# A-Nasiri-M/sap3d_tensorflow

Hardware: AMD Instinct MI355X
Metric: clips/s (16x112x112 fwd+bwd) (higher is better)
Workload: dtype f32

## Files before the change

### include/p3d_hip.h

```cpp
#ifndef P3D_HIP_H
#define P3D_HIP_H
#include <stddef.h>
#include <stdint.h>

#ifdef __cplusplus
extern "C" {
#endif

typedef struct p3d_handle p3d_handle;

enum {
    P3D_STRUCTURE_UNET = 0,
    P3D_STRUCTURE_CONCAT = 1,
    P3D_STRUCTURE_GN_P3D = 2,
    P3D_STRUCTURE_UNETPP_NONSA = 3,
    P3D_STRUCTURE_GN_P3D_DECODER = 4,
    P3D_STRUCTURE_GN_P3D_CONCAT = 5,
    P3D_STRUCTURE_UNETPP_DS = 6
};

typedef struct p3d_config {
    int structure;
    int batch;
    int frames;
// ... 104 lines not shown
typedef struct p3d_op_time {
    char name[64];
    char kernel[48];
    double ms;
    double flops;
    double bytes;
    int phase;
} p3d_op_time;
int p3d_profile_step(p3d_handle* h, float dropout_rate, uint64_t seed, p3d_op_time* out, int cap);

#define P3D_COMM_ID_BYTES 128
int p3d_comm_unique_id(void* id_out);
int p3d_comm_init(p3d_handle* h, const void* id);
int p3d_device_count(void);
int p3d_comm_info(p3d_handle* h, int* n_ranks, int* rank, int* device);
int p3d_debug_bucket_audit(p3d_handle* h, float dropout_rate, uint64_t seed, int64_t bucket_floats, int64_t* lo, int64_t* hi,
                           int32_t* after_op, int cap, int64_t* n_train, int64_t* stale);

int64_t p3d_debug_dirty_counters(void);

int p3d_debug_install_abort_trace(void);

int p3d_debug_force_plan(int igemm_tile, int igemm_splits, int wgrad_tm, int wgrad_tn);

int p3d_op_conv3d(int device, const float* x, const int64_t xshape[5], const float* w, const int64_t wshape[5],
                  const int s[3], const float* bias, float* y);
int p3d_op_conv3d_backprop_input(int device, const float* dy, const float* w, const int64_t wshape[5],
                                 const int s[3], const int64_t xshape[5], float* dx);
int p3d_op_conv3d_backprop_filter(int device, const float* x, const int64_t xshape[5], const float* dy,
                                  const int64_t wshape[5], const int s[3], float* dw, float* dbias);
int p3d_op_conv3d_transpose(int device, const float* x, const int64_t xshape[5], const float* k,
                            const int64_t kshape[5], const int s[3], const float* bias, float* y);
int p3d_debug_stem_wgrad_through_bn(int device, const float* x, const int64_t xshape[5], const float* y, const float* dz, const float* tab,
                                    const float* coef, int batch, float* dw_fused, float* dw_two_launches);
int p3d_debug_conv_bn_stats(int device, const float* x, const int64_t xshape[5], const float* w, const float* w2, const int64_t wshape[5],
                            const int s[3], const float* bias, int transpose, float* moving, float* y, float* y2, float* stats,
                            int* nparts, const char** kernel);
int p3d_debug_bn_pass(int device, int mode, int64_t M, int C, const float* y1, int ld1, int off1, const float* y2, int ld2, int off2,
                      const float* params, int batch1, int batch2, int update_moving, const float* dz, int acc2, float drop_rate,
                      uint64_t seed, int seed_dev, int path, float* z, int ldz, int offz, float* dy1, float* dy2, float* grads,
                      float* moving, int* info);
int p3d_debug_gn_pass(int device, int mode, int N, int R, int C, int G, float eps, const float* y1, int ld1, const float* y2, int ld2,
                      int ldz, const float* params, const float* cs, const float* ss, const float* dz, int acc2, float drop_rate,
                      uint64_t seed, int path, float* z, float* dy1, float* dy2, float* grads, float* tables, int* info);
int p3d_debug_cbam(int device, int N, int D, int H, int W, int C, const float* x, int ld, const float* k0, const float* b0,
                   const float* k1, const float* b1, const float* k7, int chunks, const float* dout, int accx, float* cs, float* sp,
                   float* ss, float* dx, float* pgrads, int* info);
int p3d_debug_head(int device, int transpose, int N, int D, int H, int W, int C, const float* x, const float* k, const float* bias,
                   int sigmoid, const float* dlogits, int fwd_path, int filter_path, float* logits, float* pred, float* dx, float* dk,
                   float* dbias, int* info);
int p3d_debug_smooth_l1(int device, const float* pred, const float* target, int64_t n, int through_sigmoid, int offset, double* loss,
                        float* dlogits, int* info);
int p3d_debug_loss(int device, int kind, const float* logits, const float* pred, const float* target, int64_t n, int through_sigmoid,
                   int offset, double* loss, float* dlogits, int* info);
int p3d_debug_map_loss(int device, const float* logits, const float* pred, const float* target, int64_t maps, int64_t map_elems,
                       int through_sigmoid, int offset, float kld_weight, float cc_weight, double* loss, float* dlogits,
                       double* per_map, int* info);
int p3d_debug_saliency_loss(int device, const float* logits, const float* pred, const float* target, const unsigned char* fix,
                            int64_t maps, int64_t map_elems, int through_sigmoid, int offset, float kld_weight, float cc_weight,
                            float nss_weight, float sim_weight, double* loss, float* dlogits, double* per_map, int* info);
int p3d_debug_adam_decay(int device, float* p, float* g, float* m, float* v, int64_t n, int offset, const int64_t* tile_off,
                         const int64_t* tile_len, const float* tile_c, int ntile, float lr, int64_t t, float b1, float b2, float eps,
                         int lr_on_device, int update, double* term, float* lr_t);
int p3d_debug_adam(int device, float* p, const float* g, float* m, float* v, int64_t n, int offset, float lr, int64_t t, float b1,
                   float b2, float eps, int lr_on_device, float* lr_t);
int p3d_debug_optimizer(int device, int kind, float* p, float* g, float* m, int64_t n, int offset, float lr, float momentum,
                        int use_nesterov, int lr_on_device);
int p3d_debug_optimizer_decay(int device, int kind, float* p, float* g, float* m, int64_t n, int offset, const int64_t* tile_off,
                              const int64_t* tile_len, const float* tile_c, int ntile, float lr, float momentum, int use_nesterov,
                              int lr_on_device, int update, double* term);
int p3d_debug_ema(int device, float* s, const float* p, int64_t n, int offset, float om, int om_on_device);
int p3d_debug_grad_accum(int device, int mode, float* acc, float* g, int64_t n, int offset);
int p3d_debug_augment(int device, const float* x, const float* y, const unsigned char* fix, int B, int T, int H, int W, const int32_t* geom,
                      const float* photo, int offset, float* x_out, float* y_out, unsigned char* fix_out);
int p3d_debug_augment_draw(uint64_t seed, uint64_t g, int H, int W, const p3d_augment* cfg, int32_t geom[6], float photo[2]);
int p3d_debug_opt_scaled(int device, int kind, float* p, float* g, float* m, float* v, int64_t n, int offset, const int64_t* tile_off,
                         const int64_t* tile_len, const float* tile_c, int ntile, float lr, int64_t t, float b1, float b2, float eps,
                         float momentum, int use_nesterov, int lr_on_device, float gscale, double* term, float* lr_t);
int p3d_debug_grad_norm(int device, const float* g, const float* p, int64_t n, int offset, const int64_t* chunk_off,
                        const int64_t* chunk_len, const float* chunk_c, int nchunk, const int64_t* range_lo, const int64_t* range_hi,
                        int nrange, float clip_norm, int max_blocks, double* sumsq, double* norm, float* scale);
int p3d_debug_stat_parts(const int64_t xshape[5], const int64_t wshape[5], const int s[3], int transpose, int* written, int* cap);
int p3d_debug_igemm_groupable(const int64_t xshape[5], const int64_t wshape[5], const int s[3]);
int p3d_op_max_pool3d(int device, const float* x, const int64_t xshape[5], const int ksize[3], const int s[3], float* y);
int p3d_op_max_pool3d_grad(int device, const float* x, const int64_t xshape[5], const int ksize[3], const int s[3],
                           const float* dy, float* dx);
int p3d_op_bias_add_grad(int device, const float* dy, int64_t rows, int channels, float* dbias);
int p3d_debug_conv_launch(int device, int kind, const float* in, int ld_in, int off_in, const int64_t xshape[5], const float* w,
                          const int64_t wshape[5], const int s[3], const float* bias, int accum, int f16, float* out, int ld_out,
                          int off_out, char* kernels, int kernels_cap, int* splits);
int p3d_debug_wgrad_group(int device, int n, const float* const* x, const int* ldx, const int* offx, const int64_t* xs,
                          const float* const* dy, const int* lddy, const int* offdy, const int64_t* ws, const int* s, const int* transpose,
                          float* const* dw, float* const* dbias, int polite, int greedy, char* kernel, int kernel_cap, int* cuts,
                          int* info);
typedef struct p3d_fused_bn {
    const float* y; int ld, off;
    const float* gamma; const float* beta;
    const float* partials; int nparts; int64_t rows; int publish, update_moving;
    float* scale; float* shift; float* mean; float* invstd;
    float* moving_mean; float* moving_var;
} p3d_fused_bn;
typedef struct p3d_fused_bn_grad {
    const float* y; int ld, off;
    const float* gamma; const float* mean; const float* invstd;
    const float* partials; int nparts; int64_t rows; int publish;
    float* coef; float* dgamma; float* dbeta;
} p3d_fused_bn_grad;
typedef struct p3d_fused_gate {
    const float* y; int ld_y, off_y;
    const float* scale; const float* shift; const float* mean; const float* invstd;
    float* out; int ld_out, off_out;
    float* part; int part_rows;
} p3d_fused_gate;
typedef struct p3d_fused_conv {
    int kind;
    int64_t xshape[5]; int64_t wshape[5]; int stride[3];
    const float* w; const float* bias; int f16;
    int at; p3d_fused_bn src[2];
    const float* g; int ld_g, off_g;
    int grad; p3d_fused_bn_grad gbn;
    int ngate; p3d_fused_gate gate[2]; int raw_store, accum;
    float* out; int ld_out, off_out;
    int gpart_rows;
} p3d_fused_conv;
int p3d_debug_fused_conv(int device, p3d_fused_conv* a, char* kernels, int kernels_cap, int* splits);
int p3d_debug_fused_wgrad(int device, int n, const float* const* x, const int* ldx, const int* offx, const int64_t* xs,
                          const float* const* dy, const int* lddy, const int* offdy, const int64_t* ws, const int* s,
                          const int* xt, const float* const* x2, const int* ldx2, const int* offx2, const float* const* xs1,
                          const float* const* xt1, const float* const* xs2, const float* const* xt2, const int* dyt,
                          const float* const* dy2, const int* lddy2, const int* offdy2, const float* const* dcoef,
                          float* const* dw, float* const* dbias, char* kernel, int kernel_cap, int* cuts, int* info);
int p3d_debug_fused_reject(int device, int which, int* error, int* validator);
int p3d_debug_max_pool3d(int device, const float* x, int ldx, int offx, const int64_t xshape[5], const int ksize[3], const int s[3],
                         float* y, int ldy, int offy);
int p3d_debug_max_pool3d_grad(int device, const float* x, int ldx, int offx, const int64_t xshape[5], const int ksize[3], const int s[3],
                              const float* dy, int ldy, int offy, int accumulate, float* dx, const char** kernel);
int p3d_debug_bias_add_grad(int device, const float* dy, int64_t rows, int channels, int ld, int off, float* dbias);
int p3d_op_attention_core(int device, int batch, int n_g, int n_f, int ch, const float* g, const float* f, const float* h,
                          float* o, const float* d_o, float* dg, float* df, float* dh);
int p3d_debug_attention_core(int device, int mode, int batch, int n_g, int n_f, int ch, const float* g, const float* f, const float* h,
                             float* o, const float* d_o, float* dg, float* df, float* dh);
int p3d_debug_attention_splits(int batch, int n_g, int n_f, int ch, int splits[4]);
int p3d_debug_softmax_rows(int device, int backward, int64_t rows, int cols, int ld, float* s, float* d, int guard_rows);
int p3d_debug_attn_mix(int device, int64_t M, int C, const float* r, int ldr, int offr, const float* x, int ldx, int offx, float gamma,
                       float drop_rate, uint64_t seed, int seed_dev, float* z, int ldz, int offz, const float* dz, int accx, float* dr,
                       float* dx, float* dgamma);

int p3d_metric_cc(int device, const float* map1, const float* map2, int n_maps, int n_pix, double* out);
int p3d_metric_sim(int device, const float* map1, const float* map2, int n_maps, int n_pix, double* out);
int p3d_metric_nss(int device, const float* sal, const float* fix, int n_maps, int n_pix, double* out);
int p3d_metric_auc_judd(int device, const float* sal, const float* fix, const float* jitter, int n_maps, int n_pix, double* out);
int p3d_metric_auc_borji(int device, const float* sal, const float* fix, const int* rand_idx, int n_pix, int n_fix, int n_rep,
                         double step_size, double* out);
int p3d_mapf_frames(int device, const unsigned char* bgr, int n, int H0, int W0, const float mean_rgb[3], int H, int W, float* out);
int p3d_mapf_density(int device, const unsigned char* grey, int n, int H0, int W0, int H, int W, float* out);

int p3d_resize_linear(int device, const float* src, int n, int h, int w, int H, int W, float* dst);
int p3d_metric_auc_shuffled(int device, const float* sal, const float* fix, const int* other_idx, int n_pix, int n_fix, int n_rand,
                            int n_rep, double step_size, double* out);
int p3d_eval_last_frames(p3d_handle* h, const unsigned char* density, int Hd, int Wd, const unsigned char* fixation, int H, int W,
                         const double* jitter, const int* borji_idx, const int* n_fix, int n_rep, double step_size, double* out,
                         double* stage_ms);
int p3d_debug_eval_maps(int device, const float* maps, int n_maps, int h, int w, int elem_stride, const unsigned char* density,
                        int Hd, int Wd, const unsigned char* fixation, int H, int W, const double* jitter, const int* borji_idx,
                        const int* n_fix, int n_rep, double step_size, double* out);

// ... 233 lines not shown
```

### sap3d_tensorflow_amd/csrc/conv_igemm2.hip

```cpp
#if !defined(__gfx950__) && !defined(__gfx942__) && defined(__HIP_DEVICE_COMPILE__)
#error "the K-slice exchange (write-through slab stores + relaxed ticket + one-lane acquire) is written for gfx942 / gfx950 cache semantics"
#endif
#include "p3d_kernels.h"
#include "igemm_epilogue.h"
#include <algorithm>
#include <cstddef>
#include <cstdio>
#include <cstring>
#include <cstdlib>
#include <map>
#include <mutex>
#include <tuple>
#include <vector>

typedef float f32x16 __attribute__((ext_vector_type(16)));
typedef unsigned u32x4 __attribute__((ext_vector_type(4)));

namespace {

constexpr int BK = 32;
#ifndef P3D_RING64
#define P3D_RING64 3
#endif
template <int BM, int BN>
struct Ring { static constexpr int stages = (BM >= 128) ? 2 : P3D_RING64; };

template <int AT>
struct ATr {
    static constexpr bool two = (AT == P3D_AT_RELU2 || AT == P3D_AT_GRAD);
    static constexpr int ncoef = AT == P3D_AT_RELU1 ? 2 : AT == P3D_AT_RELU2 ? 4 : AT == P3D_AT_GRAD ? 3 : 0;
};

__device__ __forceinline__ void glds16(const float* gsrc, float* lds_wave_base) {
    __builtin_amdgcn_global_load_lds((const __attribute__((address_space(1))) void*)gsrc,
                                     (__attribute__((address_space(3))) void*)lds_wave_base, 16, 0, 0);
}

template <int N>
__device__ __forceinline__ void wait_vmcnt() {
    asm volatile("s_waitcnt vmcnt(%0)" ::"n"(N) : "memory");
}

template <int LA, bool TWO>
struct ALoad {
    int base[LA];
    int dhw[LA];
    const float* aptr[LA];
    const float* aptr2[TWO ? LA : 1];
    int achunk[LA];
    int t, kc;
    int issued;
};
template <int LB>
struct BLoad {
    int boff[LB];
    int bk[LB];
    bool bok[LB];
    int t, kc, issued;
    const float* w;
};

template <int BM, bool TWO>
__device__ __forceinline__ void a_init(const IgemmArgs& p, const Geo& geo, ALoad<BM / 32, TWO>& st, unsigned m0, unsigned M, int wave, int lane,
                                       int s_begin, int kchunks) {
    constexpr int LA = BM / 32;
    const int a_slot = lane & 7, a_sub = lane >> 3;
#pragma unroll
    for (int i = 0; i < LA; ++i) {
        const int r = (i * 4 + wave) * 8 + a_sub;
        const unsigned m = m0 + r;
        st.base[i] = -1; st.dhw[i] = 0; st.aptr[i] = nullptr;
        if (TWO) st.aptr2[TWO ? i : 0] = nullptr;
        st.achunk[i] = 4 * (a_slot ^ ((r >> 1) & 7));
        if (m < M) {
            const unsigned t1 = p3d_div(m, geo.fGw), gw = m - t1 * (unsigned)geo.Gw;
            const unsigned t2 = p3d_div(t1, geo.fGh), gh = t1 - t2 * (unsigned)geo.Gh;
            const unsigned n = p3d_div(t2, geo.fGd), gd = t2 - n * (unsigned)geo.Gd;
            st.base[i] = (int)n * p.Di * p.Hi * p.Wi;
            st.dhw[i] = (int)(((gd * p.isd) << 20) | ((gh * p.ish) << 10) | (gw * p.isw));
        }
    }
    st.t = s_begin / kchunks; st.kc = s_begin - st.t * kchunks; st.issued = 0;
}
template <int BN, bool WT>
__device__ __forceinline__ void b_init(const IgemmArgs& p, const float* w, BLoad<BN / 32>& st, int n0, int wave, int lane, int s_begin, int kchunks) {
    constexpr int LB = BN / 32;
    st.w = w;
    const int a_slot = lane & 7, a_sub = lane >> 3;
    if (!WT) {
        constexpr int LANES_PER_ROW = BN / 4, ROWS_PER_PIECE = 64 / LANES_PER_ROW;
#pragma unroll
        for (int i = 0; i < LB; ++i) {
            const int kr = (i * 4 + wave) * ROWS_PER_PIECE + lane / LANES_PER_ROW;
            const int nc = n0 + (lane % LANES_PER_ROW) * 4;
            st.bk[i] = kr; st.bok[i] = nc < p.Nc; st.boff[i] = kr * p.Nc + nc;
        }
    } else {
#pragma unroll
        for (int i = 0; i < LB; ++i) {
            const int r = (i * 4 + wave) * 8 + a_sub;
            st.bk[i] = 4 * (a_slot ^ ((r >> 1) & 7));
            st.bok[i] = (n0 + r) < p.Nc;
            st.boff[i] = (n0 + r) * p.K + st.bk[i];
        }
    }
    st.t = s_begin / kchunks; st.kc = s_begin - st.t * kchunks; st.issued = 0;
}

template <int LA, bool TWO>
__device__ __forceinline__ void a_set_tap(const IgemmArgs& p, P3dKTap* taps, ALoad<LA, TWO>& st) {
    const P3dTap tap = p3d_ktap(taps, st.t);
#pragma unroll
    for (int i = 0; i < LA; ++i) {
        const int id = (st.dhw[i] >> 20) + tap.dd, ih = ((st.dhw[i] >> 10) & 1023) + tap.dh, iw = (st.dhw[i] & 1023) + tap.dw;
        const bool ok = st.base[i] >= 0 && (unsigned)id < (unsigned)p.Di && (unsigned)ih < (unsigned)p.Hi &&
                        (unsigned)iw < (unsigned)p.Wi;
        const long long row = (long long)st.base[i] + ((long long)id * p.Hi + ih) * p.Wi + iw;
        st.aptr[i] = ok ? p.x + row * p.ldx + st.achunk[i] : nullptr;
        if (TWO) st.aptr2[TWO ? i : 0] = ok ? p.x2 + row * p.ldx2 + st.achunk[i] : nullptr;
    }
}

template <int BM>
__device__ __forceinline__ void issue_a_dma(const IgemmArgs& p, P3dKTap* taps, float* __restrict__ a_dst, ALoad<BM / 32, false>& st, int nsteps,
                                            int kchunks, bool first, int wave, int lane) {
    constexpr int LA = BM / 32;
    const bool live = st.issued < nsteps;
    if (live && (first || st.kc == 0)) a_set_tap(p, taps, st);
    const int k0 = st.kc * BK;
    const float* zp = p.zeros + 4 * (lane & 7);
#pragma unroll
    for (int i = 0; i < LA; ++i) {
        const bool ok = live && st.aptr[i] != nullptr && (k0 + st.achunk[i]) < p.K;
        glds16(ok ? st.aptr[i] + k0 : zp, a_dst + (i * 4 + wave) * 8 * BK);
    }
    ++st.issued;
    if (++st.kc == kchunks) { st.kc = 0; ++st.t; }
}
template <int BN, bool WT>
__device__ __forceinline__ void issue_b_dma(const IgemmArgs& p, P3dKTap* taps, float* __restrict__ b_dst, BLoad<BN / 32>& st, int nsteps, int kchunks,
                                            int wave, int lane) {
    constexpr int LB = BN / 32;
    const bool live = st.issued < nsteps;
    const int k0 = st.kc * BK;
    const float* zp = p.zeros + 4 * (lane & 7);
    const float* wt = st.w + (long long)taps[live ? st.t : 0].widx * p.K * p.Nc;
    if (!WT) {
#pragma unroll
        for (int i = 0; i < LB; ++i) {
            const bool ok = live && st.bok[i] && (k0 + st.bk[i]) < p.K;
            glds16(ok ? wt + (long long)k0 * p.Nc + st.boff[i] : zp, b_dst + (i * 4 + wave) * 256);
        }
    } else {
#pragma unroll
        for (int i = 0; i < LB; ++i) {
            const bool ok = live && st.bok[i] && (k0 + st.bk[i]) < p.K;
            glds16(ok ? wt + k0 + st.boff[i] : zp, b_dst + (i * 4 + wave) * 8 * BK);
        }
    }
    ++st.issued;
    if (++st.kc == kchunks) { st.kc = 0; ++st.t; }
}

struct AMeta {
    unsigned ok;
    int k0;
};
template <int BM, int AT>
__device__ __forceinline__ void issue_a_raw(const IgemmArgs& p, P3dKTap* taps, float* __restrict__ raw_dst, float* __restrict__ raw2_dst, AMeta& r,
                                            ALoad<BM / 32, ATr<AT>::two>& st, int nsteps, int kchunks, bool first, int wave, int lane) {
    constexpr int LA = BM / 32;
    constexpr bool TWO = ATr<AT>::two;
    const bool live = st.issued < nsteps;
    if (live && (first || st.kc == 0)) a_set_tap(p, taps, st);
    const int k0 = st.kc * BK;
    const float* zp = p.zeros + 4 * (lane & 7);
    r.ok = 0; r.k0 = k0;
#pragma unroll
    for (int i = 0; i < LA; ++i) {
        const bool ok = live && st.aptr[i] != nullptr && (k0 + st.achunk[i]) < p.K;
        r.ok |= (ok ? 1u : 0u) << i;
        glds16(ok ? st.aptr[i] + k0 : zp, raw_dst + (i * 4 + wave) * 8 * BK);
        if (TWO) glds16(ok ? st.aptr2[TWO ? i : 0] + k0 : zp, raw2_dst + (i * 4 + wave) * 8 * BK);
    }
    ++st.issued;
    if (++st.kc == kchunks) { st.kc = 0; ++st.t; }
}
__device__ __forceinline__ float relu_nan(float v) { return v > 0.f ? v : (v != v ? v : 0.f); }
__device__ __forceinline__ float4 relu_affine4(float4 s, float4 u, float4 t) {
    return make_float4(relu_nan(fmaf(s.x, u.x, t.x)), relu_nan(fmaf(s.y, u.y, t.y)), relu_nan(fmaf(s.z, u.z, t.z)),
                       relu_nan(fmaf(s.w, u.w, t.w)));
}
template <int LA, int AT>
struct XIn {
    float4 u[LA];
    float4 v[ATr<AT>::two ? LA : 1];
    float4 c[LA][ATr<AT>::ncoef];
};
template <int BM, int AT>
__device__ __forceinline__ void transform_load(const AMeta& r, const float* __restrict__ raw_src, const float* __restrict__ raw2_src,
                                               const int (&achunk)[BM / 32], const float* __restrict__ tab, int kp,
// ... 170 lines not shown
template <int BM, int BN, bool WT, bool F16, int AT, int K>
struct FusedLoop {
    static __device__ __forceinline__ void run(const IgemmArgs& p, P3dKTap* taps, float* ring, const float* tab, int kp, f32x16 (&acc)[BM / 64][BN / 64],
                                               AMeta (&meta)[Ring<BM, BN>::stages - 1], ALoad<BM / 32, ATr<AT>::two>& sa,
                                               BLoad<BN / 32>& sb, int base, int nsteps, int kchunks, int wave, int lane, int wm, int wn) {
        using L = Lds<BM, BN, AT>;
        constexpr int S = L::STAGES, PERIOD = S * (S - 1);
        if constexpr (K < PERIOD) {
            if (base + K < nsteps) {
                constexpr int RS = (K + 1) % (S - 1);
                pipe_step_fused<BM, BN, WT, F16, AT>(p, taps, ring + ((K + 1) % 2) * L::A_STAGE, ring + L::B_OFF + ((K + S - 1) % S) * L::B_STAGE,
                                                     ring + L::RAW_OFF + RS * L::A_STAGE, ring + L::RAW2_OFF + RS * L::A_STAGE,
                                                     ring + (K % 2) * L::A_STAGE, ring + L::B_OFF + (K % S) * L::B_STAGE, tab, kp, acc,
                                                     meta[RS], sa, sb, nsteps, kchunks, wave, lane, wm, wn);
            }
            FusedLoop<BM, BN, WT, F16, AT, K + 1>::run(p, taps, ring, tab, kp, acc, meta, sa, sb, base, nsteps, kchunks, wave, lane, wm, wn);
        }
    }
};

__device__ __forceinline__ void fold_partials(const float* part_base, int nparts, int C, int k, double& s1, double& s2) {
    const float2* part = reinterpret_cast<const float2*>(part_base) + k;
    float2 v[P3D_FOLD_MAX];
#pragma unroll
    for (int q = 0; q < P3D_FOLD_MAX; ++q) v[q] = part[(size_t)min(q, nparts - 1) * C];
#pragma unroll
    for (int q = 0; q < P3D_FOLD_MAX; ++q)
        if (q < nparts) { s1 += (double)v[q].x; s2 += (double)v[q].y; }
}
__device__ __forceinline__ void bn_fold_channel(const BnFold& f, int k, bool owner, float& sc, float& sh) {
    if (!f.part) { sc = f.scale[k]; sh = f.shift[k]; return; }
    double s1 = 0.0, s2 = 0.0;
    fold_partials(f.part, f.nparts, f.C, k, s1, s2);
    const double mean = s1 * f.inv_m;
    double var = s2 * f.inv_m - mean * mean;
    if (var < 0.0) var = 0.0;
    const float meanf = (float)mean, varf = (float)var;
    const float inv = 1.0f / sqrtf(varf + f.eps);
    sc = f.gamma[k] * inv;
    sh = f.beta[k] - meanf * sc;
    if (owner && f.publish) {
        f.scale[k] = sc; f.shift[k] = sh; f.mean[k] = meanf; f.invstd[k] = inv;
        if (f.update_moving) {
            f.moving_mean[k] -= (f.moving_mean[k] - meanf) * (1.0f - 0.99f);
            f.moving_var[k] -= (f.moving_var[k] - varf) * (1.0f - 0.99f);
        }
    }
}
__device__ __forceinline__ void bn_grad_fold_channel(const BnGradFold& f, int k, bool owner, float& k1, float& k2, float& k3) {
    if (!f.part) { k1 = f.coef[k]; k2 = f.coef[f.C + k]; k3 = f.coef[2 * f.C + k]; return; }
    double sg = 0.0, sgx = 0.0;
    fold_partials(f.part, f.nparts, f.C, k, sg, sgx);
    const float inv = f.invstd[k];
    const float c1 = (float)(sg * f.inv_m), c2 = (float)(sgx * f.inv_m);
    k1 = f.gamma[k] * inv;
    k2 = -k1 * inv * c2;
    k3 = -k1 * c1 - k2 * f.mean[k];
    if (owner && f.publish) {
        f.coef[k] = k1; f.coef[f.C + k] = k2; f.coef[2 * f.C + k] = k3;
        f.dgamma[k] = (float)sgx; f.dbeta[k] = (float)sg;
    }
}

template <int AT>
__device__ __forceinline__ void build_table(const IgemmArgs& p, float* tab, int kp, bool owner) {
    for (int k = threadIdx.x; k < kp; k += 256) {
        if constexpr (AT == P3D_AT_RELU1 || AT == P3D_AT_RELU2) {
            float s = 0.f, t = 0.f;
            if (k < p.K) bn_fold_channel(p.f1, k, owner, s, t);
            tab[k] = s; tab[kp + k] = t;
            if constexpr (AT == P3D_AT_RELU2) {
                float s2 = 0.f, t2 = 0.f;
                if (k < p.K) bn_fold_channel(p.f2, k, owner, s2, t2);
                tab[2 * kp + k] = s2; tab[3 * kp + k] = t2;
            }
        } else if constexpr (AT == P3D_AT_GRAD) {
            float k1 = 0.f, k2 = 0.f, k3 = 0.f;
            if (k < p.K) bn_grad_fold_channel(p.gf, k, owner, k1, k2, k3);
            tab[k] = k1; tab[kp + k] = k2; tab[2 * kp + k] = k3;
        }
    }
}

template <int BM, int BN, bool WT, bool F16, int AT>
__device__ __forceinline__ void igemm2_body(const IgemmArgs& p, const Geo& geo, const int tile_id, const int slice) {
    constexpr int TM = BM / 64, TN = BN / 64;
    constexpr int LA = BM / 32;
    using L = Lds<BM, BN, AT>;
    constexpr int STAGES = L::STAGES;

    P3D_CHAIN_PRIO();
    extern __shared__ __attribute__((aligned(16))) char smem[];
    int* rowIdx = reinterpret_cast<int*>(smem);
    float* ring = reinterpret_cast<float*>(rowIdx + BM);
    float* tab = ring + L::FIXED;

    const int tid = threadIdx.x;
    const int lane = tid & 63;
    const int wave = __builtin_amdgcn_readfirstlane(tid >> 6);
    const int wm = wave >> 1, wn = wave & 1;
    const int h = lane >> 5, l31 = lane & 31;

    const long long M = (long long)p.N * geo.Gd * geo.Gh * geo.Gw;
    const int NT = (p.Nc + BN - 1) / BN;
    const int nsplit = geo.nsplit;
    P3dKTap* taps = geo.taps;
    const int nt = tile_id % NT;
    const int mt = tile_id / NT;
    const long long m0 = (long long)mt * BM;
    const int n0 = nt * BN;
    const int kchunks = (p.K + BK - 1) / BK;
    const int kp = kchunks * BK;
    const float4 bias4 = igemm_bias_prefetch<BN>(geo.bias, n0, p.Nc);

    const unsigned Mu = (unsigned)M, m0u = (unsigned)m0;
    auto fill_row_table = [&]() {
        for (int r = tid; r < BM; r += 256) {
            const unsigned m = m0u + r;
            int ro = -1;
            if (m < Mu) {
                const unsigned t1 = p3d_div(m, geo.fGw), gw = m - t1 * (unsigned)geo.Gw;
                const unsigned t2 = p3d_div(t1, geo.fGh), gh = t1 - t2 * (unsigned)geo.Gh;
                const unsigned n = p3d_div(t2, geo.fGd), gd = t2 - n * (unsigned)geo.Gd;
                const int od = gd * p.osd + geo.ood, oh = gh * p.osh + geo.ooh, ow = gw * p.osw + geo.oow;
                ro = (((int)n * p.Do + od) * p.Ho + oh) * p.Wo + ow;
            }
            rowIdx[r] = ro;
        }
    };
    const int total_steps = geo.ntaps * kchunks;
    const int per = (total_steps + nsplit - 1) / nsplit;
    const int s_begin = slice * per;
    const int s_end = min(total_steps, s_begin + per);
    const int nsteps = max(s_end - s_begin, 0);

    f32x16 acc[TM][TN];
#pragma unroll
    for (int i = 0; i < TM; ++i)
#pragma unroll
        for (int j = 0; j < TN; ++j)
#pragma unroll
            for (int e = 0; e < 16; ++e) acc[i][j][e] = 0.f;

    ALoad<LA, ATr<AT>::two> sa;
    BLoad<BN / 32> sb;
    a_init<BM, ATr<AT>::two>(p, geo, sa, m0u, Mu, wave, lane, s_begin, kchunks);
    b_init<BN, WT>(p, geo.w, sb, n0, wave, lane, s_begin, kchunks);
    if constexpr (AT == P3D_AT_NONE) {
#pragma unroll
        for (int k = 0; k < STAGES - 1; ++k) {
            issue_a_dma<BM>(p, taps, ring + k * L::A_STAGE, sa, nsteps, kchunks, k == 0, wave, lane);
            issue_b_dma<BN, WT>(p, taps, ring + L::B_OFF + k * L::B_STAGE, sb, nsteps, kchunks, wave, lane);
        }
        fill_row_table();
        for (int base = 0; base < nsteps; base += STAGES)
            StepLoop<BM, BN, WT, F16, 0>::run(p, taps, ring, acc, sa, sb, base, nsteps, kchunks, wave, lane, wm, wn);
    } else {
        AMeta meta[STAGES - 1];
        float* raw = ring + L::RAW_OFF;
        float* raw2 = ring + L::RAW2_OFF;
        fill_row_table();
        issue_a_raw<BM, AT>(p, taps, raw, raw2, meta[0], sa, nsteps, kchunks, true, wave, lane);
        if constexpr (STAGES == 3) {
            issue_a_raw<BM, AT>(p, taps, raw + L::A_STAGE, raw2 + L::A_STAGE, meta[1], sa, nsteps, kchunks, false, wave, lane);
            issue_b_dma<BN, WT>(p, taps, ring + L::B_OFF, sb, nsteps, kchunks, wave, lane);
        }
        build_table<AT>(p, tab, kp, tile_id == 0 && slice == 0);
        wait_vmcnt<0>();
        __syncthreads();
        {
            XIn<LA, AT> xin;
            transform_load<BM, AT>(meta[0], raw, raw2, sa.achunk, tab, kp, xin, wave, lane);
            transform_store<BM, AT>(meta[0], xin, ring, wave, lane);
        }
        issue_a_raw<BM, AT>(p, taps, raw, raw2, meta[0], sa, nsteps, kchunks, false, wave, lane);
        issue_b_dma<BN, WT>(p, taps, ring + L::B_OFF + (STAGES - 2) * L::B_STAGE, sb, nsteps, kchunks, wave, lane);
        for (int base = 0; base < nsteps; base += STAGES * (STAGES - 1))
            FusedLoop<BM, BN, WT, F16, AT, 0>::run(p, taps, ring, tab, kp, acc, meta, sa, sb, base, nsteps, kchunks, wave, lane, wm, wn);
    }

    constexpr int LDT = BN + 4;
    constexpr int F4R = BN / 4;
    float* tile = ring;
    float* sred = tile + BM * LDT;
    int* flag = reinterpret_cast<int*>(sred + 2 * 4 * BN * 2);
    wait_vmcnt<0>();
    __syncthreads();
#pragma unroll
    for (int i = 0; i < TM; ++i)
#pragma unroll
        for (int j = 0; j < TN; ++j)
#pragma unroll
            for (int e = 0; e < 16; ++e) {
                const int r = wm * (BM / 2) + i * 32 + (e & 3) + 8 * (e >> 2) + 4 * h;
                tile[r * LDT + wn * (BN / 2) + j * 32 + l31] = acc[i][j][e];
            }
    __syncthreads();

    if (nsplit > 1) {
        float* myslab = geo.slab + ((size_t)tile_id * nsplit + slice) * (BM * BN);
        const auto rs = __builtin_amdgcn_make_buffer_rsrc(myslab, 0, BM * BN * 4, 0x00020000);
#pragma unroll 4
        for (int i = tid; i < BM * F4R; i += 256) {
            const int r = i / F4R, c4 = (i - r * F4R) * 4;
            const float4 v = *reinterpret_cast<const float4*>(tile + r * LDT + c4);
            const u32x4 u = {__float_as_uint(v.x), __float_as_uint(v.y), __float_as_uint(v.z), __float_as_uint(v.w)};
            __builtin_amdgcn_raw_buffer_store_b128(u, rs, (r * BN + c4) * 4, 0, 16);
        }
        wait_vmcnt<0>();
        __syncthreads();
        if (tid == 0) {
            const unsigned ticket = __hip_atomic_fetch_add(geo.cnt + tile_id, 1u, __ATOMIC_RELAXED, __HIP_MEMORY_SCOPE_AGENT);
            const int last = ticket == (unsigned)(nsplit - 1);
            if (last) {
                __builtin_amdgcn_fence(__ATOMIC_ACQUIRE, "agent");
                asm volatile("s_waitcnt vmcnt(0)" ::: "memory");
                geo.cnt[tile_id] = 0;
            }
            *flag = last;
        }
        __syncthreads();
        if (!*flag) return;
        const float* slabs = geo.slab + (size_t)tile_id * nsplit * (BM * BN);
        constexpr int PER_LANE = BM * F4R / 256;
        static_assert(PER_LANE % 4 == 0, "reducer unrolls four tile positions");
#pragma unroll 1
        for (int i0 = 0; i0 < PER_LANE; i0 += 4) {
            float4 v[4];
            const float* src[4];
#pragma unroll
            for (int q = 0; q < 4; ++q) {
                const int i = tid + (i0 + q) * 256;
                const int r = i / F4R, c4 = (i - r * F4R) * 4;
                src[q] = slabs + r * BN + c4;
                v[q] = *reinterpret_cast<const float4*>(src[q]);
            }
            int sidx = 1;
            for (; sidx + 3 < nsplit; sidx += 4) {
                float4 a[4][4];
#pragma unroll
                for (int t = 0; t < 4; ++t)
#pragma unroll
                    for (int q = 0; q < 4; ++q) a[t][q] = *reinterpret_cast<const float4*>(src[q] + (size_t)(sidx + t) * (BM * BN));
#pragma unroll
                for (int t = 0; t < 4; ++t)
#pragma unroll
                    for (int q = 0; q < 4; ++q) { v[q].x += a[t][q].x; v[q].y += a[t][q].y; v[q].z += a[t][q].z; v[q].w += a[t][q].w; }
            }
            for (; sidx < nsplit; ++sidx) {
                float4 a[4];
#pragma unroll
                for (int q = 0; q < 4; ++q) a[q] = *reinterpret_cast<const float4*>(src[q] + (size_t)sidx * (BM * BN));
#pragma unroll
                for (int q = 0; q < 4; ++q) { v[q].x += a[q].x; v[q].y += a[q].y; v[q].z += a[q].z; v[q].w += a[q].w; }
            }
#pragma unroll
            for (int q = 0; q < 4; ++q) {
                const int i = tid + (i0 + q) * 256;
                const int r = i / F4R, c4 = (i - r * F4R) * 4;
                *reinterpret_cast<float4*>(tile + r * LDT + c4) = v[q];
            }
        }
        __syncthreads();
    }

    igemm_tile_epilogue<BM, BN>(p, geo, tile, sred, rowIdx, mt, n0, M, bias4);
}

__device__ __forceinline__ int xcd_tile(int b, int T, int min_tiles) {
    if (T < min_tiles) return b;
    const int x = b & 7, q = T >> 3, r = T & 7;
    return x * q + min(x, r) + (b >> 3);
}

template <int BM, int BN, bool WT, bool F16 = false, int AT = 0>
__global__ __launch_bounds__(256) void igemm2_kernel(const IgemmArgs p) {
    p3d_warm_kernargs<IgemmArgs>();
    Geo geo;
    geo.Gd = p.Gd; geo.Gh = p.Gh; geo.Gw = p.Gw; geo.fGd = p.fGd; geo.fGh = p.fGh; geo.fGw = p.fGw;
    geo.ood = p.ood; geo.ooh = p.ooh; geo.oow = p.oow; geo.stat_base = p.stat_base; geo.ntaps = p.ntaps; geo.taps = p3d_kernarg_taps(offsetof(IgemmArgs, taps));
    geo.w = p.w; geo.bias = p.bias; geo.y = p.y; geo.statpart = p.statpart;
    geo.nsplit = p.nsplit; geo.slab = p.slab; geo.cnt = p.cnt;
    const int tile = p.nsplit == 1 ? xcd_tile((int)blockIdx.x, (int)gridDim.x, p.xcd_min_tiles) : (int)blockIdx.x;
    igemm2_body<BM, BN, WT, F16, AT>(p, geo, tile, (int)blockIdx.y);
}
template <int BM, int BN, bool WT, bool F16 = false>
__global__ __launch_bounds__(256) void igemm2_group_kernel(const IgemmGroupArgs g) {
    p3d_warm_kernargs<IgemmArgs>();
    int c = 0;
#pragma unroll
    for (int q = 1; q < P3D_IGEMM_CLASSES; ++q)
        if (q < g.nclass && (int)blockIdx.x >= g.cls[q].blk0) c = q;
    Geo geo;
    geo.Gd = g.cls[c].Gd; geo.Gh = g.cls[c].Gh; geo.Gw = g.cls[c].Gw; geo.fGd = g.cls[c].fGd; geo.fGh = g.cls[c].fGh; geo.fGw = g.cls[c].fGw;
    geo.ood = g.cls[c].ood; geo.ooh = g.cls[c].ooh; geo.oow = g.cls[c].oow; geo.stat_base = g.cls[c].stat_base; geo.ntaps = g.cls[c].ntaps;
    geo.taps = p3d_kernarg_taps(offsetof(IgemmGroupArgs, cls) + (size_t)c * sizeof(IgemmClass) + offsetof(IgemmClass, taps));
    geo.w = g.cls[c].w; geo.bias = g.cls[c].bias; geo.y = g.cls[c].y; geo.statpart = g.cls[c].statpart;
    const int tile0 = g.cls[c].tile0;
    geo.nsplit = g.cls[c].nsplit;
    geo.slab = g.common.slab + (g.cls[c].slab0 - (long long)tile0 * geo.nsplit * (BM * BN));
    geo.cnt = g.common.cnt + (g.cls[c].cnt0 - tile0);
    const int local = (int)blockIdx.x - g.cls[c].blk0;
    const int tile = geo.nsplit == 1 ? xcd_tile(local, g.cls[c].ntiles, g.common.xcd_min_tiles) : local / geo.nsplit;
    igemm2_body<BM, BN, WT, F16, 0>(g.common, geo, tile0 + tile, local % geo.nsplit);
}

constexpr int MAX_TABLE_FLOATS = 4 * 2048;

template <int BM, int BN, int AT>
constexpr size_t smem_fixed_bytes() { return (size_t)BM * 4 + (size_t)Lds<BM, BN, AT>::FIXED * 4; }

template <int BM, int BN, bool WT, bool F16, int AT>
hipError_t launch_variant(const IgemmArgs& a, dim3 grid, hipStream_t s) {
    constexpr size_t fixed = smem_fixed_bytes<BM, BN, AT>();
    static std::once_flag once;
    std::call_once(once, [] {
        hipFuncSetAttribute((const void*)igemm2_kernel<BM, BN, WT, F16, AT>, hipFuncAttributeMaxDynamicSharedMemorySize,
                            (int)(fixed + (AT ? MAX_TABLE_FLOATS * 4 : 0)));
    });
    const size_t kp = (size_t)((a.K + BK - 1) / BK) * BK;
    const size_t sm = fixed + (size_t)ATr<AT>::ncoef * kp * 4;
    hipLaunchKernelGGL((igemm2_kernel<BM, BN, WT, F16, AT>), grid, dim3(256), sm, s, a);
    return hipGetLastError();
}

int xcd_min_tiles() {
    static const int v = [] { const char* e = p3d_tune_env("P3D_TUNE_XCD_MIN_TILES"); return e ? atoi(e) : 64; }();
    return v;
}
bool tail_split_enabled() {
    static const bool on = [] { const char* e = p3d_tune_env("P3D_TUNE_NO_TAIL"); return !(e && atoi(e)); }();
    return on;
}
int tail_slices(long long rem, int steps, int bm, int bn) {
    if (rem <= 0 || !tail_split_enabled()) return 1;
    const double step_us = bm * bn == 16384 ? 2.3 : (bm * bn == 8192 ? 1.35 : 0.78);
    const double whole = steps * step_us;
    double best = whole * 0.9;
    int best_s = 1;
    for (int sl = 2; sl <= 16 && steps / sl >= 4; ++sl) {
        const long long rounds = (rem * sl + 255) / 256;
        const double cost = (double)rounds * ((steps + sl - 1) / sl) * step_us + 3.0 + 0.4 * sl;
        if (cost < best) { best = cost; best_s = sl; }
    }
    return best_s;
}

template <int BM, int BN>
hipError_t launch_t(const IgemmArgs& a0, const P3dIgemmPlan& pl, hipStream_t s) {
    IgemmArgs a = a0;
    const long long M = (long long)a.N * a.Gd * a.Gh * a.Gw;
    const long long tiles = ((M + BM - 1) / BM) * ((a.Nc + BN - 1) / BN);
    const int splits = pl.splits < 1 ? 1 : pl.splits;
    a.nsplit = splits;
    a.xcd_min_tiles = xcd_min_tiles();
    a.slab = nullptr; a.cnt = nullptr;
    if (splits > 1) {
        const hipError_t e = p3d_stream_scratch(s, (size_t)tiles * splits * BM * BN, (size_t)tiles, &a.slab, &a.cnt);
        if (e != hipSuccess) return e;
    }
    const dim3 grid((unsigned)tiles, (unsigned)splits);
    if (a.wT) {
        if (a.at_mode == P3D_AT_GRAD) return a.f16 ? launch_variant<BM, BN, true, true, P3D_AT_GRAD>(a, grid, s) : launch_variant<BM, BN, true, false, P3D_AT_GRAD>(a, grid, s);
        if (a.at_mode != P3D_AT_NONE) return hipErrorInvalidValue;
        return a.f16 ? launch_variant<BM, BN, true, true, 0>(a, grid, s) : launch_variant<BM, BN, true, false, 0>(a, grid, s);
    }
    switch (a.at_mode) {
        case P3D_AT_NONE: return a.f16 ? launch_variant<BM, BN, false, true, 0>(a, grid, s) : launch_variant<BM, BN, false, false, 0>(a, grid, s);
        case P3D_AT_RELU1: return a.f16 ? launch_variant<BM, BN, false, true, P3D_AT_RELU1>(a, grid, s) : launch_variant<BM, BN, false, false, P3D_AT_RELU1>(a, grid, s);
        case P3D_AT_RELU2: return a.f16 ? launch_variant<BM, BN, false, true, P3D_AT_RELU2>(a, grid, s) : launch_variant<BM, BN, false, false, P3D_AT_RELU2>(a, grid, s);
        default: return hipErrorInvalidValue;
    }
}

struct Scratch { float* slab = nullptr; size_t slab_floats = 0; unsigned* cnt = nullptr; size_t counters = 0; };
std::vector<void*> g_scratch_allocs;
std::map<hipStream_t, Scratch> g_scratch;
std::mutex g_scratch_mutex;

}

hipError_t p3d_stream_scratch(hipStream_t s, size_t slab_floats, size_t counters, float** slab, unsigned** cnt) {
    std::lock_guard<std::mutex> g(g_scratch_mutex);
    Scratch& sc = g_scratch[s];
    if (slab_floats > sc.slab_floats) {
        const size_t want = slab_floats + slab_floats / 2 + (1u << 20);
        float* p = nullptr;
// ... 173 lines not shown
        hipFuncSetAttribute((const void*)igemm2_group_kernel<BM, BN, false, false>, hipFuncAttributeMaxDynamicSharedMemorySize, (int)sm);
        hipFuncSetAttribute((const void*)igemm2_group_kernel<BM, BN, true, false>, hipFuncAttributeMaxDynamicSharedMemorySize, (int)sm);
        hipFuncSetAttribute((const void*)igemm2_group_kernel<BM, BN, false, true>, hipFuncAttributeMaxDynamicSharedMemorySize, (int)sm);
        hipFuncSetAttribute((const void*)igemm2_group_kernel<BM, BN, true, true>, hipFuncAttributeMaxDynamicSharedMemorySize, (int)sm);
    });
    const dim3 grid((unsigned)blocks), blk(256);
    const IgemmArgs& a = g.common;
    if (a.f16) {
        if (a.wT) hipLaunchKernelGGL((igemm2_group_kernel<BM, BN, true, true>), grid, blk, sm, s, g);
        else hipLaunchKernelGGL((igemm2_group_kernel<BM, BN, false, true>), grid, blk, sm, s, g);
    } else {
        if (a.wT) hipLaunchKernelGGL((igemm2_group_kernel<BM, BN, true, false>), grid, blk, sm, s, g);
        else hipLaunchKernelGGL((igemm2_group_kernel<BM, BN, false, false>), grid, blk, sm, s, g);
    }
    return hipGetLastError();
}
}


bool p3d_igemm2_tail_split(const IgemmArgs& a, const P3dIgemmPlan& pl) {
    if (a.at_mode || a.ngate || pl.splits > 1 || pl.stream_blocks > 0 || !tail_split_enabled()) return false;
    const long long M = (long long)a.N * a.Gd * a.Gh * a.Gw;
    const long long tiles = ((M + pl.bm - 1) / pl.bm) * ((a.Nc + pl.bn - 1) / pl.bn);
    const int steps = a.ntaps * ((a.K + BK - 1) / BK);
    return tiles >= 256 && tail_slices(tiles % 256, steps, pl.bm, pl.bn) >= 2;
}

hipError_t p3d_launch_igemm2_group(const IgemmArgs* v, int n, const P3dIgemmPlan& pl, hipStream_t s) {
    if (n == 1 ? !p3d_igemm2_tail_split(v[0], pl) : !p3d_igemm2_groupable(v, n, pl)) return hipErrorInvalidValue;
    for (int i = 0; i < n; ++i) {
        const IgemmArgs& a = v[i];
        const long long M = (long long)a.N * a.Gd * a.Gh * a.Gw;
        if (M >= (1ll << 31) || (long long)a.N * a.Di * a.Hi * a.Wi >= (1ll << 31) || (long long)a.N * a.Do * a.Ho * a.Wo >= (1ll << 31))
            return hipErrorInvalidValue;
        if (a.Gd * a.isd >= 1024 || a.Gh * a.ish >= 1024 || a.Gw * a.isw >= 1024 || a.ntaps > P3D_MAX_TAPS) return hipErrorInvalidValue;
        if ((a.K & 3) || (a.ldx & 3) || !a.zeros || (a.Nc & 3) || (a.ldy & 3)) return hipErrorInvalidValue;
    }
    int order[P3D_IGEMM_CLASSES];
    for (int i = 0; i < n; ++i) order[i] = i;
    std::stable_sort(order, order + n, [&](int x, int y) { return v[x].ntaps > v[y].ntaps; });
    IgemmGroupArgs g;
    memset(&g, 0, sizeof(g));
    g.common = v[0];
    g.common.xcd_min_tiles = xcd_min_tiles();
    g.common.nsplit = 1; g.common.slab = nullptr; g.common.cnt = nullptr;
    long long tiles[P3D_IGEMM_CLASSES];
    int nc = 0;
    for (int k = 0; k < n; ++k) {
        const IgemmArgs& a = v[order[k]];
        const long long M = (long long)a.N * a.Gd * a.Gh * a.Gw;
        if (M <= 0) continue;
        IgemmClass& c = g.cls[nc];
        c.Gd = a.Gd; c.Gh = a.Gh; c.Gw = a.Gw;
        c.fGd = p3d_fastdiv((unsigned)a.Gd); c.fGh = p3d_fastdiv((unsigned)a.Gh); c.fGw = p3d_fastdiv((unsigned)a.Gw);
        c.ood = a.ood; c.ooh = a.ooh; c.oow = a.oow; c.stat_base = a.stat_base; c.ntaps = a.ntaps;
        c.w = a.w; c.bias = a.bias; c.y = a.y; c.statpart = a.statpart;
        c.nsplit = std::max(1, p3d_igemm2_plan(a, 1).splits);
        for (int t = 0; t < a.ntaps; ++t) c.taps[t] = a.taps[t];
        tiles[nc] = ((M + pl.bm - 1) / pl.bm) * ((a.Nc + pl.bn - 1) / pl.bn);
        ++nc;
    }
    if (nc >= 1 && nc < P3D_IGEMM_CLASSES && g.cls[nc - 1].nsplit == 1) {
        long long blocks = 0;
        for (int q = 0; q < nc; ++q) blocks += tiles[q] * g.cls[q].nsplit;
        const long long rem = blocks % 256;
        const IgemmClass& last = g.cls[nc - 1];
        const int steps = last.ntaps * ((g.common.K + BK - 1) / BK);
        const int sl = tail_slices(rem, steps, pl.bm, pl.bn);
        if (blocks >= 256 && rem > 0 && rem < tiles[nc - 1] && sl >= 2) {
            g.cls[nc] = last;
            g.cls[nc].tile0 = (int)(tiles[nc - 1] - rem);
            g.cls[nc].nsplit = sl;
            tiles[nc] = rem;
            tiles[nc - 1] -= rem;
            ++nc;
        }
    }
    g.nclass = nc;
    if (nc == 0) return hipSuccess;
    if (pl.bm == 128 && pl.bn == 128) return launch_group_t<128, 128>(g, tiles, s);
    if (pl.bm == 128 && pl.bn == 64) return launch_group_t<128, 64>(g, tiles, s);
    return launch_group_t<64, 64>(g, tiles, s);
}
```

### sap3d_tensorflow_amd/csrc/igemm_epilogue.h

```cpp
#pragma once
#include "p3d_kernels.h"

typedef const P3dTap __attribute__((address_space(4))) P3dKTap;
__device__ __forceinline__ P3dKTap* p3d_kernarg_taps(size_t byte_offset) {
    typedef const char __attribute__((address_space(4))) kchar_t;
    return (P3dKTap*)((kchar_t*)__builtin_amdgcn_kernarg_segment_ptr() + byte_offset);
}
__device__ __forceinline__ P3dTap p3d_ktap(P3dKTap* taps, int i) {
    P3dTap t;
    t.dd = taps[i].dd; t.dh = taps[i].dh; t.dw = taps[i].dw; t.widx = taps[i].widx;
    return t;
}
struct Geo {
    int Gd, Gh, Gw;
    P3dFastDiv fGd, fGh, fGw;
    int ood, ooh, oow, stat_base, ntaps;
    P3dKTap* taps;
    const float* w; const float* bias; float* y; float* statpart;
    int nsplit; float* slab; unsigned* cnt;
};

__device__ __forceinline__ float4 shfl_xor4(float4 v, int o) {
    return make_float4(__shfl_xor(v.x, o), __shfl_xor(v.y, o), __shfl_xor(v.z, o), __shfl_xor(v.w, o));
}

template <int BN>
__device__ __forceinline__ float4 igemm_bias_prefetch(const float* bias, int n0, int Nc) {
    const int col = n0 + ((int)threadIdx.x % (BN / 4)) * 4;
    return (bias && col < Nc) ? *reinterpret_cast<const float4*>(bias + col) : make_float4(0.f, 0.f, 0.f, 0.f);
}
template <int BM, int BN>
__device__ __forceinline__ void igemm_tile_epilogue(const IgemmArgs& p, const Geo& geo, float* tile, float* sred, const int* rowIdx,
                                                    const int mt, const int n0, const long long M, const float4 bias4) {
    constexpr int LDT = BN + 4;
    constexpr int F4R = BN / 4;
    const int tid = threadIdx.x;
    const int lane = tid & 63;
    const int wave = __builtin_amdgcn_readfirstlane(tid >> 6);
    if (p.ngate > 0) {
        const int c4 = (tid % F4R) * 4, col = n0 + c4;
        const bool cok = col < p.Nc;
        float4 sc[2], sh[2], mu[2], iv[2], s[2], sx[2];
#pragma unroll
        for (int q = 0; q < 2; ++q) {
            s[q] = make_float4(0.f, 0.f, 0.f, 0.f); sx[q] = s[q]; sc[q] = s[q]; sh[q] = s[q]; mu[q] = s[q]; iv[q] = s[q];
            if (q < p.ngate && cok) {
                sc[q] = *reinterpret_cast<const float4*>(p.gate[q].scale + col); sh[q] = *reinterpret_cast<const float4*>(p.gate[q].shift + col);
                mu[q] = *reinterpret_cast<const float4*>(p.gate[q].mean + col); iv[q] = *reinterpret_cast<const float4*>(p.gate[q].invstd + col);
            }
        }
#pragma unroll 2
        for (int r = tid / F4R; r < BM; r += 256 / F4R) {
            const int ro = rowIdx[r];
            if (ro < 0 || !cok) continue;
            float4 v = *reinterpret_cast<const float4*>(tile + r * LDT + c4);
            v.x += bias4.x; v.y += bias4.y; v.z += bias4.z; v.w += bias4.w;
            if (p.accum) { const float4 o = *reinterpret_cast<const float4*>(geo.y + (long long)ro * p.ldy + col); v.x += o.x; v.y += o.y; v.z += o.z; v.w += o.w; }
            if (p.raw_store) *reinterpret_cast<float4*>(geo.y + (long long)ro * p.ldy + col) = v;
#pragma unroll
            for (int q = 0; q < 2; ++q) {
                if (q >= p.ngate) break;
                const float4 y4 = *reinterpret_cast<const float4*>(p.gate[q].y + (long long)ro * p.gate[q].ldy + col);
                float4 g;
                g.x = fmaf(sc[q].x, y4.x, sh[q].x) > 0.f ? v.x : 0.f; g.y = fmaf(sc[q].y, y4.y, sh[q].y) > 0.f ? v.y : 0.f;
                g.z = fmaf(sc[q].z, y4.z, sh[q].z) > 0.f ? v.z : 0.f; g.w = fmaf(sc[q].w, y4.w, sh[q].w) > 0.f ? v.w : 0.f;
                *reinterpret_cast<float4*>(p.gate[q].out + (long long)ro * p.gate[q].ldo + col) = g;
                s[q].x += g.x; s[q].y += g.y; s[q].z += g.z; s[q].w += g.w;
                sx[q].x = fmaf(g.x, (y4.x - mu[q].x) * iv[q].x, sx[q].x); sx[q].y = fmaf(g.y, (y4.y - mu[q].y) * iv[q].y, sx[q].y);
                sx[q].z = fmaf(g.z, (y4.z - mu[q].z) * iv[q].z, sx[q].z); sx[q].w = fmaf(g.w, (y4.w - mu[q].w) * iv[q].w, sx[q].w);
            }
        }
        __syncthreads();
#pragma unroll
        for (int q = 0; q < 2; ++q) {
            if (q >= p.ngate) break;
#pragma unroll
            for (int o = F4R; o < 64; o <<= 1) {
                const float4 a = shfl_xor4(s[q], o), b = shfl_xor4(sx[q], o);
                s[q].x += a.x; s[q].y += a.y; s[q].z += a.z; s[q].w += a.w;
                sx[q].x += b.x; sx[q].y += b.y; sx[q].z += b.z; sx[q].w += b.w;
            }
            if (lane < F4R) {
                float* d = sred + ((q * 4 + wave) * BN + c4) * 2;
                d[0] = s[q].x; d[1] = sx[q].x; d[2] = s[q].y; d[3] = sx[q].y; d[4] = s[q].z; d[5] = sx[q].z; d[6] = s[q].w; d[7] = sx[q].w;
            }
        }
        __syncthreads();
        if (tid < BN && (n0 + tid) < p.Nc) {
#pragma unroll
            for (int q = 0; q < 2; ++q) {
                if (q >= p.ngate) break;
                float t1 = 0.f, t2 = 0.f;
#pragma unroll
                for (int w = 0; w < 4; ++w) { t1 += sred[((q * 4 + w) * BN + tid) * 2]; t2 += sred[((q * 4 + w) * BN + tid) * 2 + 1]; }
                float* dst = p.gate[q].part + ((size_t)mt * p.Nc + n0 + tid) * 2;
                dst[0] = t1; dst[1] = t2;
            }
        }
        return;
    }

    const bool want_stats = geo.statpart != nullptr;
// ... 33 lines not shown
```

### sap3d_tensorflow_amd/csrc/net.hip

```cpp
#include "../../include/p3d_hip.h"
#include "p3d_kernels.h"

#include <rccl/rccl.h>

#include <algorithm>
#include <atomic>
#include <cmath>
#include <cstdio>
#include <cstring>
#include <deque>
#include <functional>
#include <map>
#include <memory>
#include <mutex>
#include <stdexcept>
#include <string>
#include <vector>

namespace {

thread_local std::string g_err;

struct RuntimeEnv { bool debug_sync = false, graph = false, no_side_stream = false; };
const RuntimeEnv& runtime_env() {
// ... 266 lines not shown
        static const char* const tiles[3] = {"64,64", "128,64", "128,128"};
        static const char* const ats[4] = {"", ",relu1", ",relu2", ",bngrad"};
        static std::map<int, std::string> names;
        const int key = (pl.bm == 128 ? (pl.bn == 128 ? 2 : 1) : 0) * 8 + a.at_mode * 2 + (a.ngate ? 1 : 0);
        std::string& nm = names[key];
        if (nm.empty()) nm = std::string("igemm2_kernel<") + tiles[key / 8] + ats[a.at_mode] + (a.ngate ? ",gate" : "") + ">";
        name = nm.c_str();
    }
    launch(c, name, fl, by, [&]() { return p3d_launch_igemm2(a, pl, c.s); });
}

void zero_strided(const Ctx& c, float* p, int ld, int64_t rows, int C);

struct StatSink { float* part = nullptr; int cap = 0; int* nparts = nullptr; };

int bn_part_cap(int64_t rows, int C) {
    return (int)std::max<int64_t>({rows / 64 + 80, (int64_t)p3d_bn_stats_parts((long)rows, C), (int64_t)p3d_pw_stream_max_blocks(rows, C)});
}

void launch_igemm_group(const Ctx& c, std::vector<IgemmArgs>& v, const P3dIgemmPlan& pl, const char* suffix) {
    double fl = 0, by = 0;
    for (auto& a : v) { double f1, b1; igemm_work(a, f1, b1); fl += f1; by += b1; }
    const std::string kn = "igemm2_group_kernel<" + std::to_string(pl.bm) + "," + std::to_string(pl.bn) + ">" + suffix;
    launch(c, kn.c_str(), fl, by, [&]() { return p3d_launch_igemm2_group(v.data(), (int)v.size(), pl, c.s); });
}

void run_igemm_group(const Ctx& c, std::vector<IgemmArgs>& v, bool accumulate, const StatSink* stats, hipEvent_t fork = nullptr,
                     hipEvent_t join = nullptr) {
    int base = 0;
    for (auto& a : v) {
        a.accum = accumulate ? 1 : 0;
        a.statpart = nullptr; a.stat_base = 0;
        a.zeros = g_zero_page;
        if (stats && stats->part) {
            const P3dIgemmPlan pl = p3d_igemm2_plan(a, 1);
            const int mt = p3d_igemm2_mtiles(a, pl);
            if (base + mt > stats->cap) throw P3dError("statistics partials overflow their arena slot");
            a.statpart = stats->part; a.stat_base = base;
            base += mt;
        }
    }
    if (v.size() >= 2 && !c.dry) {
        const P3dIgemmPlan pl = p3d_igemm2_plan(v[0], 1);
        if (p3d_igemm2_groupable(v.data(), (int)v.size(), pl)) {
            launch_igemm_group(c, v, pl, "");
            if (stats && stats->nparts) *stats->nparts = base;
            return;
        }
    }
    const bool spread = fork && join && c.side && !c.dry && !c.prof && v.size() >= 4;
    Ctx sc = c;
    if (spread) {
        sc.s = c.side;
        HIPCHECK(ev_record(fork, c.s));
        HIPCHECK(ev_wait(c.side, fork));
    }
    int index = 0;
    for (auto& a : v) {
        launch_igemm((spread && (index & 1)) ? sc : c, a, 1);
        ++index;
    }
    if (spread) {
        HIPCHECK(ev_record(join, c.side));
        HIPCHECK(ev_wait(c.s, join));
    }
    if (stats && stats->nparts) *stats->nparts = base;
}

void sibling_prepare(IgemmArgs& a, const StatSink* sink) {
    a.zeros = g_zero_page; a.accum = 0; a.statpart = nullptr; a.stat_base = 0;
    if (!sink) return;
    const int mt = p3d_igemm2_mtiles(a, p3d_igemm2_plan(a, 1));
    if (mt > sink->cap) throw P3dError("statistics partials overflow their arena slot");
    a.statpart = sink->part; *sink->nparts = mt;
}
bool launch_siblings(const Ctx& c, std::vector<IgemmArgs>& v) {
    const P3dIgemmPlan pl = p3d_igemm2_plan(v[0], 1);
    if (p3d_igemm2_groupable(v.data(), (int)v.size(), pl)) {
        launch_igemm_group(c, v, pl, "(siblings)");
        return true;
    }
    for (auto& q : v) launch_igemm(c, q, 1);
    return false;
}

float adam_step_size(float lr, float b1, float b2, int64_t t_step) {
    const double t = (double)t_step;
    return (float)(lr * std::sqrt(1.0 - std::pow((double)b2, t)) / (1.0 - std::pow((double)b1, t)));
}

template <typename Args>
void set_dropout(Args& a, const Ctx& c, bool dropout) {
    if (dropout && c.training && c.drop > 0.f) { a.drop_rate = c.drop; a.drop_scale = 1.f / (1.f - c.drop); a.seed = c.seed; a.seed_dev = c.seed_dev; }
}

GnParams gn_layout(const float* gamma, const float* beta, double* sums, float* tab, int N, int C, int G) {
    GnParams p;
    const int64_t nc = (int64_t)N * C;
    p.gamma = gamma; p.beta = beta; p.sums = sums; p.C = C; p.G = G;
    p.scale = tab; p.shift = tab + nc; p.mean = tab + 2 * nc; p.invstd = tab + 3 * nc; p.coef = tab + 4 * nc;
    return p;
}
struct GnOperand {
    const float* y = nullptr; int ld = 0; float* dy = nullptr; int lddy = 0;
    GnParams g = {}; float* dgamma = nullptr; float* dbeta = nullptr;
};
GnApplyArgs gn_apply_args(int mode, int64_t M, int R, int C, float eps, const GnOperand& o1, const GnOperand& o2, int acc2,
                          const float* cs, const float* ss, float* z, int ldz, const float* dz, const Ctx& c, bool dropout) {
    GnApplyArgs a;
    memset(&a, 0, sizeof(a));
    a.mode = mode; a.M = M; a.R = R; a.C = C;
    a.y1 = o1.y; a.ld1 = o1.ld; a.g1 = o1.g; a.dy1 = o1.dy; a.lddy1 = o1.lddy; a.dgamma1 = o1.dgamma; a.dbeta1 = o1.dbeta;
    a.y2 = o2.y; a.ld2 = o2.ld; a.g2 = o2.g; a.dy2 = o2.dy; a.lddy2 = o2.lddy; a.dgamma2 = o2.dgamma; a.dbeta2 = o2.dbeta; a.acc2 = acc2;
    a.cs = cs; a.ss = ss; a.z = z; a.ldz = ldz; a.dz = dz; a.eps = eps;
    set_dropout(a, c, dropout);
    return a;
}

bool gn_small_rule(int mode, int R, int C, int G1, int G2, bool dropout) {
    static const bool no_small = p3d_tune_env("P3D_NO_GN_SMALL") != nullptr;
    return !no_small && mode != 2 && !dropout && p3d_gn_small_ok(R, C, G1) && (!G2 || G2 == G1);
}
void gn_pass_forward(const Ctx& c, const GnApplyArgs& a, bool small) {
    const double tens = (double)a.M * a.C * 4.0;
    const int R = a.R, C = a.C, N = (int)(a.M / a.R), io = a.y2 ? 3 : 2;
    if (small) {
        const std::string ksf = "gn_small_fwd_kernel<" + std::to_string(a.mode) + ">";
        launch(c, ksf.c_str(), 0, tens * io, [&]() { return p3d_gn_small_fwd(a, c.s); });
        return;
    }
    const std::string ka = "gn_apply_kernel<" + std::to_string(a.mode) + ">";
    launch(c, "gn_stats_kernel", 0, tens, [&]() { return p3d_gn_stats(a.y1, a.ld1, N, R, C, a.g1.sums, c.s); });
    launch(c, "gn_finalize_kernel", 0, 32.0 * N * C, [&]() { return p3d_gn_finalize(a.g1, N, R, a.eps, c.s); });
    if (a.mode == 2 || a.mode == 3) {
        launch(c, "gn_stats_kernel", 0, tens, [&]() { return p3d_gn_stats(a.y2, a.ld2, N, R, C, a.g2.sums, c.s); });
        launch(c, "gn_finalize_kernel", 0, 32.0 * N * C, [&]() { return p3d_gn_finalize(a.g2, N, R, a.eps, c.s); });
    }
    launch(c, ka.c_str(), 0, tens * io, [&]() { return p3d_gn_apply(a, c.s); });
}
void gn_pass_backward(const Ctx& c, const GnApplyArgs& a, bool small) {
    const double tens = (double)a.M * a.C * 4.0;
    const int R = a.R, C = a.C, N = (int)(a.M / a.R);
    if (small) {
        const std::string ksb = "gn_small_bwd_kernel<" + std::to_string(a.mode) + ">";
        launch(c, ksb.c_str(), 0, tens * (a.y2 ? 5 : 3), [&]() { return p3d_gn_small_bwd(a, c.s); });
        return;
    }
    const std::string kr = "gn_bwd_reduce_kernel<" + std::to_string(a.mode) + ">";
    const std::string kb = "gn_bwd_apply_kernel<" + std::to_string(a.mode) + ">";
    launch(c, kr.c_str(), 0, tens * (a.y2 ? 3 : 2), [&]() { return p3d_gn_bwd_reduce(a, c.s); });
    launch(c, "gn_bwd_finalize_kernel", 0, 64.0 * N * C, [&]() { return p3d_gn_bwd_finalize(a.g1, N, R, a.dgamma1, a.dbeta1, c.s); });
    if (a.mode == 3)
        launch(c, "gn_bwd_finalize_kernel", 0, 64.0 * N * C, [&]() { return p3d_gn_bwd_finalize(a.g2, N, R, a.dgamma2, a.dbeta2, c.s); });
    launch(c, kb.c_str(), 0, tens * (a.y2 ? 5 : 3), [&]() { return p3d_gn_bwd_apply(a, c.s); });
}

BnParams bn_layout(const float* gamma, const float* beta, float* moving_mean, float* moving_var, float* tab, const float* statpart,
                   int nparts, int C) {
    BnParams b;
    b.gamma = gamma; b.beta = beta; b.moving_mean = moving_mean; b.moving_var = moving_var; b.statpart = statpart; b.nparts = nparts;
    b.scale = tab; b.shift = tab + C; b.mean = tab + 2 * C; b.invstd = tab + 3 * C; b.C = C;
    return b;
}

struct BnPass {
    int mode = 0; int64_t M = 0; int C = 0;
// ... 838 lines not shown
        if (wq_flushes >= wq_events.size()) {
            hipEvent_t e = nullptr;
            HIPCHECK(hipEventCreateWithFlags(&e, local_event_flags()));
            wq_events.push_back(e);
        }
        hipEvent_t ev = wq_events[wq_flushes++];
        std::vector<WgradArgs> probs;
        double fl = 0, by = 0;
        for (auto& q : wq) { probs.push_back(q.a); fl += q.flops; by += q.bytes; }
        const char* name = wgrad_group_name(probs);
        if (c.defer) {
            for (auto& pr : probs) pr.polite = 1;
            parked_flops += fl;
        }
        on_side_stream(c, ev, [=](const Ctx& sc) {
            launch_wgrad_group(sc, probs, name, fl, by);
        });
        wq.clear();
    }

    bool fuse_bn = false;
    bool fuse_bn_bwd = false;
    bool last_forward_fused = false;
    bool pred_ready = false;
    int64_t fuse_max_rows = 2048;
    struct FuseSrc { Act* y = nullptr; BN* bn = nullptr; int pub = 0; };
    struct ConvFuse {
        int at = 0;
        FuseSrc src[2];
        int ngate = 0; FuseSrc gate[2];
        Act* raw = nullptr; char* raw_flag = nullptr;
        bool accum_in = false;
        BN* out_bn = nullptr;
        bool any() const { return at != 0 || out_bn != nullptr; }
    };
    void make_fusable(BN* bn, int64_t rows) {
        if (bn->fusable) return;
        bn->fusable = true;
        reserve_stat_parts(bn, rows);
        bn->gpart_cap = (int)(rows / 64 + 8);
        bn->gpart_off = statpart_count;
        statpart_count += (int64_t)bn->gpart_cap * bn->C * 2;
        const int64_t o = bnbuf_count; bnbuf_count += 3 * (int64_t)bn->C;
        late_bind.push_back([this, bn, o]() { bn->coef = bnbuf + o; });
    }
    std::map<BN*, bool> fwd_finalized, grad_finalized;
    FusedBn fused_bn_desc(const FuseSrc& s, int64_t rows, const Ctx& c) {
        BN* bn = s.bn;
        FusedBn d;
        d.gamma = bn->gamma->p; d.beta = bn->beta->p; d.C = bn->C;
        d.scale = bn->scale; d.shift = bn->shift; d.mean = bn->mean; d.invstd = bn->invstd;
        d.moving_mean = bn->mm->p; d.moving_var = bn->mv->p;
        d.part = statpart_arena + bn->part_off; d.nparts = bn->nparts;
        d.rows = rows; d.pub = s.pub; d.update_moving = c.update_moving;
        return d;
    }
    FusedBnGrad fused_grad_desc(BN* bn, int64_t rows) {
        FusedBnGrad d;
        d.gamma = bn->gamma->p; d.mean = bn->mean; d.invstd = bn->invstd; d.C = bn->C;
        d.coef = bn->coef; d.dgamma = bn->gamma->g; d.dbeta = bn->beta->g;
        d.part = statpart_arena + bn->gpart_off; d.nparts = bn->gnparts; d.rows = rows;
        return d;
    }
    void fused_prefinalize(const Ctx& c, const ConvFuse& cf, int64_t rows) {
        if (c.dry) return;
        for (int q = 0; q < (cf.at == P3D_AT_RELU2 ? 2 : 1); ++q) {
            BN* bn = cf.src[q].bn;
            if (cf.src[q].pub != 1) continue;
            bn->used_batch = true;
            fwd_finalized[bn] = fused_bn_prefinalize(c, fused_bn_desc(cf.src[q], rows, c));
        }
    }
    BnGate bn_gate(const FuseSrc& s) {
        BnGate g;
        memset(&g, 0, sizeof(g));
        g.y = s.y->p; g.ldy = s.y->ld;
        g.scale = s.bn->scale; g.shift = s.bn->shift; g.mean = s.bn->mean; g.invstd = s.bn->invstd;
        g.out = s.y->g; g.ldo = s.y->ld;
        g.part = statpart_arena + s.bn->gpart_off;
        return g;
    }

    std::vector<IgemmArgs> sib_pending;

#include "net_ops.inc"
#include "net_gn.inc"
#include "net_graphs.inc"
#include "net_plan.inc"
#include "net_postcfg.inc"
#include "net_prior.inc"
#include "net_fixpool.inc"
#include "net_video.inc"
#include "net_trainset.inc"
#include "net_sched.inc"
};

#include "net_abi.inc"
#include "net_readout.inc"
#include "net_shots.inc"
```

### sap3d_tensorflow_amd/csrc/net_abi.inc

```
#define API_BEGIN try {
#define API_END                                        \
    }                                                  \
    catch (const std::exception& e) {                  \
        g_err = e.what();                              \
        return -1;                                     \
    }                                                  \
    return 0;

extern "C" {

const char* p3d_last_error(void) { return g_err.c_str(); }

void p3d_default_config(p3d_config* c) {
    memset(c, 0, sizeof(*c));
    c->structure = P3D_STRUCTURE_UNET;
    c->batch = 2; c->frames = 16; c->height = 112; c->width = 112; c->base = 64;
    c->blocks[0] = 3; c->blocks[1] = 8; c->blocks[2] = 36;
    c->device = 0; c->world_size = 1; c->rank = 0;
}

static void refuse_two_hip_runtimes() {
    FILE* f = fopen("/proc/self/maps", "r");
    if (!f) return;
    std::vector<std::string> seen;
// ... 706 lines not shown
    API_END
}

int p3d_set_optimizer_step(p3d_handle* h, int64_t t) {
    API_BEGIN
    if (!h) throw P3dError("null handle");
    if (t < 0) throw P3dError("optimizer step " + std::to_string(t) + " is negative");
    h->step = t;
    API_END
}

int p3d_activation_info(p3d_handle* h, const char* name, int64_t shape[5]) {
    API_BEGIN
    if (!h || !name) throw P3dError("null argument");
    auto it = h->named.find(name);
    if (it == h->named.end()) throw P3dError(std::string("no activation named ") + name);
    Act* a = it->second;
    shape[0] = a->N; shape[1] = a->D; shape[2] = a->H; shape[3] = a->W; shape[4] = a->C;
    API_END
}

int p3d_get_activation(p3d_handle* h, const char* name, float* host, int64_t count) {
    API_BEGIN
    if (!h || !name || !host) throw P3dError("null argument");
    auto it = h->named.find(name);
    if (it == h->named.end()) throw P3dError(std::string("no activation named ") + name);
    Act* a = it->second;
    if (count != a->rows() * a->C) throw P3dError("activation size mismatch");
    HIPCHECK(hipSetDevice(h->cfg.device));
    if (a->materialize && h->last_forward_fused) a->materialize(h->stream);
    h->download_act(a, host);
    API_END
}

int p3d_block_info(p3d_handle* h, int block_id, int64_t in_shape[5], int64_t out_shape[5]) {
    API_BEGIN
    if (!h) throw P3dError("null handle");
    auto it = h->blocks.find(block_id);
    if (it == h->blocks.end()) throw P3dError("no bottleneck with id " + std::to_string(block_id));
    const Act* a = it->second.in; const Act* b = it->second.out;
    if (in_shape) { in_shape[0] = a->N; in_shape[1] = a->D; in_shape[2] = a->H; in_shape[3] = a->W; in_shape[4] = a->C; }
    if (out_shape) { out_shape[0] = b->N; out_shape[1] = b->D; out_shape[2] = b->H; out_shape[3] = b->W; out_shape[4] = b->C; }
    API_END
}

int p3d_block_forward(p3d_handle* h, int block_id, const float* in, int64_t in_count, float* out, int64_t out_count) {
    API_BEGIN
    if (!h || !in || !out) throw P3dError("null argument");
    auto it = h->blocks.find(block_id);
    if (it == h->blocks.end()) throw P3dError("no bottleneck with id " + std::to_string(block_id));
    Act* a = it->second.in; Act* b = it->second.out;
    if (in_count != a->rows() * a->C || out_count != b->rows() * b->C) throw P3dError("block tensor size mismatch");
    HIPCHECK(hipSetDevice(h->cfg.device));
    HIPCHECK(hipMemcpy2DAsync(a->p, (size_t)a->ld * 4, in, (size_t)a->C * 4, (size_t)a->C * 4, (size_t)a->rows(), hipMemcpyHostToDevice, h->stream));
    Ctx c; c.training = true; c.s = h->stream; c.fuse = h->fuse_bn;
    h->last_forward_fused = c.fuse;
    h->sib_pending.clear();
    if (h->stats_count) HIPCHECK(hipMemsetAsync(h->stats_arena, 0, (size_t)h->stats_count * sizeof(double), c.s));
    for (size_t i = it->second.op0; i < it->second.op1; ++i) h->ops[i].fwd(c);
    h->download_act(b, out);
    API_END
}

int p3d_block_backward(p3d_handle* h, int block_id, const float* in, int64_t in_count, const float* dout, int64_t out_count, float* din) {
    API_BEGIN
    if (!h || !in || !dout || !din) throw P3dError("null argument");
    auto it = h->blocks.find(block_id);
    if (it == h->blocks.end()) throw P3dError("no bottleneck with id " + std::to_string(block_id));
    Act* a = it->second.in; Act* b = it->second.out;
    if (in_count != a->rows() * a->C || out_count != b->rows() * b->C) throw P3dError("block tensor size mismatch");
    if (!a->g || !b->g) throw P3dError("this bottleneck's input or output carries no gradient");
    HIPCHECK(hipSetDevice(h->cfg.device));
    HIPCHECK(hipMemcpy2DAsync(a->p, (size_t)a->ld * 4, in, (size_t)a->C * 4, (size_t)a->C * 4, (size_t)a->rows(), hipMemcpyHostToDevice, h->stream));
    Ctx c; c.training = true; c.s = h->stream; c.fuse = false;
    h->sib_pending.clear();
    h->last_forward_fused = false;
    if (h->stats_count) HIPCHECK(hipMemsetAsync(h->stats_arena, 0, (size_t)h->stats_count * sizeof(double), c.s));
    for (size_t i = it->second.op0; i < it->second.op1; ++i) h->ops[i].fwd(c);
    h->zeroed_early = false;
    h->zero_backward_arenas(c.s, true);
    c.z0 = h->zb; c.z1 = h->zb + h->zb_bytes;
    HIPCHECK(hipMemcpy2DAsync(b->g, (size_t)b->ld * 4, dout, (size_t)b->C * 4, (size_t)b->C * 4, (size_t)b->rows(), hipMemcpyHostToDevice, c.s));
    h->wq.clear(); h->wq_flushes = 0; h->parked_flops = 0;
    for (size_t i = it->second.op1; i-- > it->second.op0;) {
        c.bwd_op = h->ops[i].name.c_str();
        h->ops[i].bwd(c);
    }
    h->flush_wgrads(c);
    HIPCHECK(hipMemcpy2DAsync(din, (size_t)a->C * 4, a->g, (size_t)a->ld * 4, (size_t)a->C * 4, (size_t)a->rows(), hipMemcpyDeviceToHost, c.s));
    HIPCHECK(hipStreamSynchronize(c.s));
    API_END
}

int p3d_profile_step(p3d_handle* h, float dropout_rate, uint64_t seed, p3d_op_time* out, int cap) {
    if (!h) { g_err = "null handle"; return -1; }
    try {
        h->refuse_swapped("p3d_profile_step");
        HIPCHECK(hipSetDevice(h->cfg.device));
        PerturbPause unperturbed;
        Prof prof;
        Ctx c; c.training = true; c.drop = dropout_rate; c.seed = seed; c.update_moving = true; c.s = h->stream; c.prof = &prof;
        prof.phase = 0; h->run_forward(c);
        prof.cur_op = "loss"; h->run_loss(c);
        if (h->acc_accumulating()) {
            prof.phase = 1; h->run_backward(c, false);
            prof.phase = 2; prof.cur_op = "grad_accum"; h->grad_accum_take(c);
        } else {
            c.acc_finish = h->acc_k > 1;
            prof.phase = 1; h->run_backward(c, false);
            prof.phase = 2; prof.cur_op = "adam"; h->run_adam(c);
            h->acc_pending = 0;
        }
        HIPCHECK(hipStreamSynchronize(c.s));
        int w = 0;
        for (auto& r : prof.recs) {
            float ms = 0;
            HIPCHECK(hipEventElapsedTime(&ms, r.e0, r.e1));
            if (w < cap && out) {
                p3d_op_time& o = out[w];
                memset(&o, 0, sizeof(o));
                snprintf(o.name, sizeof(o.name), "%s", r.op.c_str());
                snprintf(o.kernel, sizeof(o.kernel), "%s", r.kernel.c_str());
                o.ms = ms; o.flops = r.flops; o.bytes = r.bytes; o.phase = r.phase;
            }
            ++w;
            hipEventDestroy(r.e0);
            hipEventDestroy(r.e1);
        }
        return w;
    } catch (const std::exception& e) {
        g_err = e.what();
        return -1;
    }
}

int p3d_debug_bucket_audit(p3d_handle* h, float dropout_rate, uint64_t seed, int64_t bucket_floats, int64_t* lo, int64_t* hi,
                           int32_t* after_op, int cap, int64_t* n_train, int64_t* stale) {
    if (!h) { g_err = "null handle"; return -1; }
    int count = 0;
    try {
        HIPCHECK(hipSetDevice(h->cfg.device));
        if (bucket_floats < 1) throw P3dError("bucket size must be positive");
        struct Snap { int64_t lo, hi; int op; std::vector<float> g; };
        std::vector<Snap> snaps;
        const int64_t saved = h->bucket_floats;
        h->bucket_floats = bucket_floats;
        h->bucket_hook = [&](int64_t l, int64_t u, int op) {
            HIPCHECK(hipStreamSynchronize(h->stream));
            HIPCHECK(hipStreamSynchronize(h->side_stream));
            Snap s; s.lo = l; s.hi = u; s.op = op; s.g.resize((size_t)(u - l));
            HIPCHECK(copy_now(s.g.data(), h->flat_g + l, (size_t)(u - l) * 4, hipMemcpyDeviceToHost, h->stream));
            snaps.push_back(std::move(s));
        };
        try {
            Ctx c; c.training = true; c.drop = dropout_rate; c.seed = seed; c.update_moving = false; c.s = h->stream;
            h->run_forward(c);
            h->run_loss(c);
            h->run_backward(c, true);
            HIPCHECK(hipStreamSynchronize(h->stream));
            HIPCHECK(hipStreamSynchronize(h->side_stream));
        } catch (...) {
            h->bucket_hook = nullptr; h->bucket_floats = saved;
            throw;
        }
        h->bucket_hook = nullptr; h->bucket_floats = saved;
        std::vector<float> fin((size_t)h->n_train);
// ... 1045 lines not shown
    if (!out) throw P3dError("null argument");
    if (mode < 0 || mode > 2) throw P3dError("perturb: mode is 0 (off), 1 (serial) or 2 (slow)");
    if (mode == 2 && (slow < 0 || slow > 1)) throw P3dError("perturb self-test: slow is 0 (the producer's stream) or 1 (the consumer's)");
    if (mode == 2 && (delay_us < 1 || delay_us > 2000)) throw P3dError("perturb: delay_us must be in [1, 2000]");
    HIPCHECK(hipSetDevice(device));
    const int n = 4096;
    struct Streams {
        int device; hipStream_t a = nullptr, b = nullptr; hipEvent_t ev = nullptr;
        explicit Streams(int d) : device(d) {
            a = take_stream(d, 0); b = take_stream(d, 0);
            HIPCHECK(hipEventCreateWithFlags(&ev, hipEventDisableTiming));
        }
        ~Streams() {
            hipStreamSynchronize(a); hipStreamSynchronize(b);
            if (ev) hipEventDestroy(ev);
            give_stream(device, 0, a); give_stream(device, 0, b);
        }
    } st(device);
    DevBuf buf(n), res(n);
    HIPCHECK(p3d_fill_uniform(buf.p, n, 1.f, 1.f, 0, st.a));
    HIPCHECK(p3d_delay(1, st.a));
    HIPCHECK(hipStreamSynchronize(st.a));
    HIPCHECK(p3d_copy_strided(res.p, 4, buf.p, 4, n / 4, 4, st.b));
    HIPCHECK(hipStreamSynchronize(st.b));
    HIPCHECK(fill_now(res.p, 0, (size_t)n * 4, st.b));
    Perturb pt;
    pt.mode = mode; pt.streams[0] = st.a; pt.streams[1] = st.b;
    if (mode == 2) { pt.target = slow ? st.b : st.a; pt.delay_us = delay_us; }
    Perturb* const before = g_perturb;
    g_perturb = mode ? &pt : nullptr;
    try {
        Ctx ca, cb; ca.s = st.a; cb.s = st.b;
        launch(ca, "fill_uniform_kernel", 0, 4.0 * n, [&]() { return p3d_fill_uniform(buf.p, n, 2.f, 2.f, 0, ca.s); });
        HIPCHECK(ev_record(st.ev, st.a));
        if (with_wait) HIPCHECK(ev_wait(st.b, st.ev));
        launch(cb, "add_inplace_kernel", 0, 8.0 * n, [&]() { return p3d_copy_strided(res.p, 4, buf.p, 4, n / 4, 4, cb.s); });
        HIPCHECK(hipStreamSynchronize(st.a));
        HIPCHECK(hipStreamSynchronize(st.b));
    } catch (...) { g_perturb = before; throw; }
    g_perturb = before;
    res.get(out, n);
    API_END
}

int p3d_debug_conv_launch(int device, int kind, const float* in, int ld_in, int off_in, const int64_t xs[5], const float* w,
                          const int64_t ws[5], const int s[3], const float* bias, int accum, int f16, float* out, int ld_out, int off_out,
                          char* kernels, int kernels_cap, int* splits) {
    API_BEGIN
    HIPCHECK(hipSetDevice(device));
    if (!in || !xs || !w || !ws || !s || !out) throw P3dError("null argument");
    if (kind < 0 || kind > 2) throw P3dError("conv_launch: kind is 0 (forward), 1 (input gradient) or 2 (transposed forward)");
    const ConvProblem p = conv_problem(xs, ws, s, kind == 2);
    if (p.stem) throw P3dError("conv_launch: the stem shape has its own entry points");
    if (kind != 2 && ws[3] != p.Cin) throw P3dError("filter Cin mismatch");
    if (kind == 2 && accum) throw P3dError("conv_launch: a transposed conv's forward never accumulates");
    if (kind == 1 && bias) throw P3dError("conv_launch: an input gradient has no bias");
    const int ntap = (int)(ws[0] * ws[1] * ws[2]);
    if (f16 && (ntap != 1 || kind == 2)) throw P3dError("conv_launch: the fp16 option is for 1x1x1 convs, forward and input gradient");
    const int64_t rin = kind == 1 ? p.rows : p.rows_in, rout = kind == 1 ? p.rows_in : p.rows;
    const int cin = kind == 1 ? p.Cout : p.Cin, cout = kind == 1 ? p.Cin : p.Cout;
    check_slice("conv_launch (gathered side)", ld_in, off_in, cin);
    check_slice("conv_launch (output side)", ld_out, off_out, cout);
    DevBuf din(rin * ld_in, in), dw(prod5(ws), w), dout(rout * ld_out, out), db(cout, bias);
    ensure_zero_page();
    const float* bp = bias ? db.p : nullptr;
    std::vector<IgemmArgs> v = kind == 1 ? p.input_gradient(din.p + off_in, dw.p, dout.p + off_out, ld_in, ld_out, accum ? 1 : 0)
                                         : p.forward(din.p + off_in, dw.p, dout.p + off_out, bp, nullptr, nullptr, ld_in, ld_out, accum ? 1 : 0);
    if (f16) for (auto& a : v) a.f16 = 1;
    Ctx c;
    std::string names;
    traced_kernels([&]() { run_igemm_group(c, v, accum != 0, nullptr); }, names);
    if (v.size() == 1 && p3d_igemm2_tail_split(v[0], p3d_igemm2_plan(v[0], 1))) names += "(tail)";
    put_string(names, kernels, kernels_cap);
    if (splits) {
        splits[0] = 1 << 30; splits[1] = 0;
        for (const IgemmArgs& a : v) {
            const P3dIgemmPlan pl = p3d_igemm2_plan(a, 1);
            const int sp = pl.stream_blocks > 0 || pl.splits < 1 ? 1 : pl.splits;
            splits[0] = std::min(splits[0], sp); splits[1] = std::max(splits[1], sp);
        }
        if (v.empty()) splits[0] = splits[1] = 0;
    }
    dout.get(out, rout * ld_out);
    API_END
}

int p3d_debug_wgrad_group(int device, int n, const float* const* x, const int* ldx, const int* offx, const int64_t* xs,
                          const float* const* dy, const int* lddy, const int* offdy, const int64_t* ws, const int* s, const int* transpose,
                          float* const* dw, float* const* dbias, int polite, int greedy, char* kernel, int kernel_cap, int* cuts,
                          int* info) {
    API_BEGIN
    HIPCHECK(hipSetDevice(device));
    if (!x || !ldx || !offx || !xs || !dy || !lddy || !offdy || !ws || !s || !transpose || !dw || !dbias || !cuts || !info)
        throw P3dError("null argument");
    if (n < 1 || n > P3D_WGRAD_GROUP) throw P3dError("wgrad_group: 1 to " + std::to_string(P3D_WGRAD_GROUP) + " problems");
    struct Bufs { std::unique_ptr<DevBuf> x, dy, dw, db; int64_t nw; int nb; };
    std::vector<Bufs> bufs((size_t)n);
    std::vector<WgradArgs> probs;
    ensure_zero_page();
    double fl = 0, by = 0;
    for (int i = 0; i < n; ++i) {
        const int64_t* xsi = xs + 5 * i; const int64_t* wsi = ws + 5 * i;
        const ConvProblem p = conv_problem(xsi, wsi, s + 3 * i, transpose[i]);
        if (p.stem) throw P3dError("wgrad_group: the stem shape has its own entry points");
        if (!transpose[i] && wsi[3] != p.Cin) throw P3dError("filter Cin mismatch");
        if (transpose[i] && dbias[i]) throw P3dError("wgrad_group: a transposed conv's bias gradient is a column sum of its own");
        check_slice("wgrad_group (x)", ldx[i], offx[i], p.Cin);
        check_slice("wgrad_group (dy)", lddy[i], offdy[i], p.Cout);
        Bufs& b = bufs[(size_t)i];
        b.nw = prod5(wsi); b.nb = p.Cout;
        b.x.reset(new DevBuf(p.rows_in * ldx[i], x[i]));
        b.dy.reset(new DevBuf(p.rows * lddy[i], dy[i]));
        if (b.nw > 0 && !dw[i]) throw P3dError("null argument");
        b.dw.reset(new DevBuf(b.nw, dw[i]));
        if (dbias[i]) b.db.reset(new DevBuf(b.nb, dbias[i]));
        WgradArgs a = p.filter_gradient(b.x->p + offx[i], ldx[i], b.dy->p + offdy[i], lddy[i], b.dw->p, dbias[i] ? b.db->p : nullptr);
        a.zeros = g_zero_page;
        a.polite = polite ? 1 : 0; a.greedy = greedy ? 1 : 0;
        double f1, b1;
        wgrad_work(a, f1, b1);
        fl += f1; by += b1;
        probs.push_back(a);
    }
    info[1] = info[2] = 0;
    if (p3d_wgrad2_group_cuts(probs.data(), n, cuts, &info[0], &info[1], &info[2]) < 0) throw P3dError("wgrad_group: a problem the kernel does not take");
    const char* name = wgrad_group_name(probs);
    put_string(name, kernel, kernel_cap);
    Ctx c;
    launch_wgrad_group(c, probs, name, fl, by);
    for (int i = 0; i < n; ++i) {
        if (bufs[(size_t)i].nw > 0) bufs[(size_t)i].dw->get(dw[i], bufs[(size_t)i].nw);
        if (dbias[i]) bufs[(size_t)i].db->get(dbias[i], bufs[(size_t)i].nb);
    }
    API_END
}

namespace {
struct InOut {
    std::unique_ptr<DevBuf> d; float* host = nullptr; int64_t n = 0;
    void put(float* h, int64_t count) { host = h; n = count; if (h) d.reset(new DevBuf(count, h)); }
    float* p() const { return d ? d->p : nullptr; }
    void back() { if (d) d->get(host, n); }
};
std::unique_ptr<DevBuf> dev_copy(const float* h, int64_t n) { return std::unique_ptr<DevBuf>(h ? new DevBuf(n, h) : nullptr); }
void report_splits(const std::vector<IgemmArgs>& v, int* splits) {
    if (!splits) return;
    splits[0] = 1 << 30; splits[1] = 0;
    for (const IgemmArgs& a : v) {
        const P3dIgemmPlan pl = p3d_igemm2_plan(a, 1);
        const int sp = pl.stream_blocks > 0 || pl.splits < 1 ? 1 : pl.splits;
        splits[0] = std::min(splits[0], sp); splits[1] = std::max(splits[1], sp);
    }
    if (v.empty()) splits[0] = splits[1] = 0;
}
}

int p3d_debug_fused_conv(int device, p3d_fused_conv* fc, char* kernels, int kernels_cap, int* splits) {
    API_BEGIN
    HIPCHECK(hipSetDevice(device));
    if (!fc || !fc->w || !fc->out) throw P3dError("null argument");
    if (fc->kind != 0 && fc->kind != 1) throw P3dError("fused_conv: kind is 0 (forward) or 1 (input gradient)");
    const ConvProblem p = conv_problem(fc->xshape, fc->wshape, fc->stride, 0);
    if (p.stem) throw P3dError("fused_conv: the stem shape has its own entry points");
    if (fc->wshape[3] != p.Cin) throw P3dError("filter Cin mismatch");
    const int ntap = (int)(fc->wshape[0] * fc->wshape[1] * fc->wshape[2]);
    if (fc->f16 && ntap != 1) throw P3dError("fused_conv: the fp16 option is for 1x1x1 convs");
// ... 432 lines not shown
```

### sap3d_tensorflow_amd/csrc/net_ops.inc

```
    Act* conv(const std::string& opname, Act* x, Param* w, Param* bias, const int k[3], const int s[3], int Cout, BN* bn,
              const std::string& out_name, bool stem = false, bool bn_has_dropout = false, int sibling = 0,
              const ConvFuse* fuse = nullptr) {
        const ConvGeo g = make_geo(x->D, x->H, x->W, k, s);
        Act* y = new_act(out_name, x->N, g.O[0], g.O[1], g.O[2], Cout);
        if (bn && stats_target(bn, y->rows(), Cout, bn_has_dropout)) reserve_stat_parts(bn, y->rows());
        const ConvFuse cf = fuse ? *fuse : ConvFuse();
        if (cf.out_bn) { if (cf.out_bn != bn) throw P3dError("fused output BatchNorm must be the conv's own"); make_fusable(bn, y->rows()); }
        fused_gate_check(s, cf.ngate);
        char* xflag = x->g ? consume(x) : nullptr;
        const int Cin = x->C;
        const int ntap = k[0] * k[1] * k[2];
        Op op;
        op.name = opname; op.kind = stem ? "conv_stem" : (ntap == 1 ? "conv_1x1x1" : "conv_kxkxk");
        op.flops = 2.0 * y->rows() * ntap * Cin * Cout;
        op.bytes = 4.0 * (x->rows() * (double)Cin + y->rows() * (double)Cout + (double)ntap * Cin * Cout);
        op.bflops = op.flops * (x->g ? 2 : 1);
        op.bbytes = op.bytes * (x->g ? 2 : 1);
        op.owns = {w}; if (bias) op.owns.push_back(bias);
        if (cf.out_bn) { op.owns.push_back(cf.out_bn->gamma); op.owns.push_back(cf.out_bn->beta); }
        hipEvent_t fork_ev = new_fork_event();
        if (stem) {
            if (k[0] != 1 || Cin != 3 || bias) throw P3dError("stem path is for [1,kh,kw,3,C] kernels without bias");
            const StemGeo sg = stem_geo(g, x->N, Cout);
            float* x4 = dalloc<float>(sg.x4_floats);
            HIPCHECK(fill_async(x4, 0, (size_t)sg.x4_floats * sizeof(float), stream, "stem-padding"));
            float* w4 = dalloc<float>(sg.w4_floats);
            float* dw4 = dalloc<float>(sg.w4_floats);
            float* spart = sg.part_floats ? dalloc<float>(sg.part_floats) : nullptr;
            auto link = std::make_shared<StemBnLink>();
            link->enabled = sg.part_floats != 0;
            y->stem_link = link;
            op.fwd = [=](const Ctx& c) {
                stem_pack(c, sg, x->p, x4, w->p, w4);
                std::vector<IgemmArgs> v{stem_forward_args(sg, x4, w4, y->p, y->ld, nullptr)};
                StatSink sink;
                run_igemm_group(c, v, false, epilogue_sink(sink, bn, y->rows(), Cout, bn_has_dropout));
            };
            op.bwd = [=](const Ctx& c) {
                const bool through_bn = link->pending;
                const BnBwdArgs bnargs = link->args;
                link->pending = false;
                on_side_stream(c, fork_ev, [=](const Ctx& sc) {
                    stem_filter_gradient(sc, sg, x4, y->g, y->ld, dw4, w->g, nullptr, true, spart, through_bn ? &bnargs : nullptr);
                });
                if (xflag) throw P3dError("the stem input carries no gradient");
            };
            ops.push_back(op);
            return y;
        }
        const auto f16 = [=] { return ntap == 1 && pointwise_f16; };
        op.fwd = [=](const Ctx& c) {
            const bool fz = c.fuse && cf.at != 0;
            if (fz) fused_prefinalize(c, cf, cf.src[0].y->rows());
            const Act* xs = fz ? cf.src[0].y : x;
            std::vector<IgemmArgs> v{igemm_conv_forward(g, x->N, xs->p, xs->ld, Cin, y->p, y->ld, Cout, w->p, bias ? bias->p : nullptr, 0)};
            IgemmArgs& a = v[0];
            StatSink sink;
            const StatSink* stats = epilogue_sink(sink, bn, y->rows(), Cout, bn_has_dropout, c.fuse && cf.out_bn);
            if (sibling && !c.dry && !fz && ntap > 0) {
                sibling_prepare(a, stats);
                if (sibling == 1) {
                    if (!sib_pending.empty()) throw P3dError("sibling conv " + opname + ": an earlier pair never sent its launch");
                    sib_pending.push_back(a);
                    return;
                }
                if (sib_pending.size() != 1) throw P3dError("sibling conv " + opname + " has no first sibling waiting");
                sib_pending.push_back(a);
                std::vector<IgemmArgs> pair;
                pair.swap(sib_pending);
                launch_siblings(c, pair);
                return;
            }
            if (fz) {
                const bool two = cf.at == P3D_AT_RELU2;
                const FusedBn s1 = fused_bn_desc(cf.src[0], cf.src[0].y->rows(), c);
                const FusedBn s2 = two ? fused_bn_desc(cf.src[1], cf.src[1].y->rows(), c) : FusedBn();
                fused_forward_operand(a, cf.at, s1, fwd_finalized[cf.src[0].bn], two ? cf.src[1].y->p : nullptr, two ? cf.src[1].y->ld : 0,
                                      two ? &s2 : nullptr, two && fwd_finalized[cf.src[1].bn]);
            }
            if (f16()) a.f16 = 1;
            run_igemm_group(c, v, false, stats);
        };
        const auto wgrad_args = [=](bool fin) {
            const Act* xs = fin ? cf.src[0].y : x;
            WgradArgs wa = wgrad_conv(g, x->N, xs->p, xs->ld, Cin, y->g, y->ld, Cout, w->g, bias ? bias->g : nullptr);
            if (fin) {
                const bool two = cf.at == P3D_AT_RELU2;
                fused_wgrad_x(wa, two ? 2 : 1, cf.src[0].bn->scale, cf.src[0].bn->shift, two ? cf.src[1].y->p : nullptr, two ? cf.src[1].y->ld : 0,
                              two ? cf.src[1].bn->scale : nullptr, two ? cf.src[1].bn->shift : nullptr);
            }
            return wa;
        };
        op.bwd = [=](const Ctx& c) {
            if (!(c.fuse_bwd && cf.any())) {
                queue_wgrad(c, wgrad_args(c.fuse && cf.at != 0));
                if (xflag) {
                    const int accum = *xflag;
                    auto v = igemm_conv_input_side(g, x->N, y->g, y->ld, Cout, x->g, x->ld, Cin, w->p, nullptr, accum,
                                                   !accum);
                    if (f16()) for (auto& a : v) a.f16 = 1;
                    run_igemm_group(c, v, accum != 0, nullptr);
                }
                return;
            }
            WgradArgs wa = wgrad_args(cf.at != 0);
            if (cf.out_bn) fused_wgrad_dy(wa, y->p, y->ld, cf.out_bn->coef);
            if (!xflag) throw P3dError("a conv with a fused BatchNorm needs an input gradient launch (it publishes the coefficients)");
            if (cf.out_bn && !c.dry) grad_finalized[cf.out_bn] = fused_bn_grad_prefinalize(c, fused_grad_desc(cf.out_bn, y->rows()));
            float* py = x->g; int pld = x->ld; int accum = *xflag;
            if (cf.ngate) {
                accum = cf.accum_in ? (int)*xflag : 0;
                if (cf.raw) { py = cf.raw->g; pld = cf.raw->ld; accum = *cf.raw_flag; }
            }
            auto v = igemm_conv_input_side(g, x->N, y->g, y->ld, Cout, py, pld, Cin, w->p, nullptr, accum, !accum);
            bool first = true;
            for (auto& a : v) {
                if (f16()) a.f16 = 1;
                if (cf.out_bn) fused_grad_operand(a, y->p, y->ld, fused_grad_desc(cf.out_bn, y->rows()), grad_finalized[cf.out_bn], first);
                first = false;
            }
            if (cf.ngate) {
                BnGate gates[2];
                for (int q = 0; q < cf.ngate; ++q) gates[q] = bn_gate(cf.gate[q]);
                const int mt = fused_gated_epilogue(v, cf.ngate, gates, cf.raw != nullptr, !c.dry);
                for (int q = 0; q < cf.ngate && !c.dry; ++q) {
                    if (mt > cf.gate[q].bn->gpart_cap) throw P3dError("gradient partials overflow their arena slot");
                    cf.gate[q].bn->gnparts = mt;
                }
            }
            run_igemm_group(c, v, accum != 0, nullptr);
            queue_wgrad(c, wa);
        };
        ops.push_back(op);
        return y;
    }

    Act* deconv(const std::string& opname, Act* x, Param* kern, Param* bias, const int k[3], const int s[3], int Cout, BN* bn,
                const std::string& out_name, bool bn_has_dropout = false) {
        const ConvGeo g = make_geo(x->D * s[0], x->H * s[1], x->W * s[2], k, s);
        Act* y = new_act(out_name, x->N, g.I[0], g.I[1], g.I[2], Cout);
        if (bn && stats_target(bn, y->rows(), Cout, bn_has_dropout)) reserve_stat_parts(bn, y->rows());
        char* xflag = x->g ? consume(x) : nullptr;
        const int Cin = x->C;
        Op op;
        op.name = opname; op.kind = "deconv";
        double taps_eff = 1;
        for (int a = 0; a < 3; ++a) taps_eff *= (double)k[a] / s[a];
        op.flops = 2.0 * y->rows() * taps_eff * Cin * Cout;
        op.bytes = 4.0 * (x->rows() * (double)Cin + y->rows() * (double)Cout + (double)k[0] * k[1] * k[2] * Cin * Cout);
        op.bflops = 2 * op.flops; op.bbytes = 2 * op.bytes;
        op.owns = {kern}; if (bias) op.owns.push_back(bias);
        hipEvent_t fork_ev = new_fork_event();
        hipEvent_t class_fork = new_fork_event(), class_join = new_fork_event();
        op.fwd = [=](const Ctx& c) {
            auto v = igemm_conv_input_side(g, x->N, x->p, x->ld, Cin, y->p, y->ld, Cout, kern->p, bias ? bias->p : nullptr,
                                           0, true);
            StatSink sink;
            run_igemm_group(c, v, false, epilogue_sink(sink, bn, y->rows(), Cout, bn_has_dropout), class_fork, class_join);
        };
        op.bwd = [=](const Ctx& c) {
            queue_wgrad(c, wgrad_conv(g, x->N, y->g, y->ld, Cout, x->p, x->ld, Cin, kern->g, nullptr));
            if (bias)
                on_side_stream(c, fork_ev, [=](const Ctx& sc) {
                    launch(sc, "colsum_kernel", 0, 4.0 * y->rows() * Cout, [&]() { return p3d_colsum(y->g, y->ld, y->rows(), Cout, bias->g, sc.s); });
                });
            if (xflag) {
                std::vector<IgemmArgs> v{igemm_conv_forward(g, x->N, y->g, y->ld, Cout, x->g, x->ld, Cin, kern->p, nullptr, *xflag)};
                run_igemm_group(c, v, *xflag != 0, nullptr);
            }
        };
        ops.push_back(op);
        return y;
    }

    Act* bn_apply(const std::string& opname, int mode, Act* y1, BN* bn1, Act* y2, BN* bn2, Act* out, const std::string& out_name,
                  bool dropout = false, bool fused_site = false) {
        if (!out) out = new_act(out_name, y1->N, y1->D, y1->H, y1->W, y1->C);
        else if (!out_name.empty()) named[out_name] = out;
        consume(y1);
        char* f2 = nullptr;
        if (y2) f2 = consume(y2);
        const bool two = (mode == 2 || mode == 3);
        const int bwd_parts = p3d_bn_bwd_parts((long)y1->rows(), y1->C);
// ... 115 lines not shown
```

### sap3d_tensorflow_amd/csrc/net_plan.inc

```
    void finalize_build() {
        flat_p = dalloc<float>(n_train); flat_g = dalloc<float>(n_train);
        flat_m = dalloc<float>(n_train); flat_v = dalloc<float>(n_train);
        flat_state = dalloc<float>(n_state);
        for (float* buf : {flat_p, flat_g, flat_m, flat_v}) HIPCHECK(fill_async(buf, 0, (size_t)n_train * 4, stream, "flat-buffer"));
        HIPCHECK(fill_now(flat_state, 0, (size_t)n_state * 4, stream));
        for (Param* p : porder) {
            if (p->trainable) { p->p = flat_p + p->off; p->g = flat_g + p->off; }
            else p->p = flat_state + p->off;
        }
        stats_arena = dalloc<double>(stats_count);
        statpart_arena = dalloc<float>(statpart_count);
        d_seed = dalloc<unsigned long long>(1);
        d_lr = dalloc<float>(1);
        d_om = dalloc<float>(1);
        red_arena = dalloc<double>(red_count);
        bnbuf = dalloc<float>(bnbuf_count);
        for (auto& f : late_bind) f();
        late_bind.clear();
        index_gradient_owners();
        for (int i = 0; i < (int)ops.size(); ++i)
            if (ops[i].name.compare(0, 5, "block") == 0) defer_release_op = i;
        if (defer_release_op == (int)ops.size() - 1) defer_release_op = -1;
        defer_budget = 0;
        if (!blocks.empty()) {
            const Act* last = blocks.rbegin()->second.out;
            if (last && last->rows() <= 2048) defer_budget = 130e9;
            if (const char* e = p3d_tune_env("P3D_TUNE_DEFER_GFLOP")) defer_budget = atof(e) * 1e9;
        }
        tune_plans();
        plan_zero_arenas();
    }

    std::vector<std::pair<int64_t, int>> own_sorted;
    std::vector<int> own_sufmin;
    void index_gradient_owners() {
        std::map<const Param*, int> owner;
        for (size_t i = 0; i < ops.size(); ++i)
            for (Param* p : ops[i].owns) {
                if (!p || !p->trainable) continue;
                if (owner.count(p)) throw P3dError("variable " + p->name + " has two gradient producers");
                owner[p] = (int)i;
            }
        for (Param* p : porder)
            if (p->trainable && !owner.count(p)) throw P3dError("variable " + p->name + " has no gradient producer");
        own_sorted.clear();
        for (auto& kv : owner) own_sorted.push_back({kv.first->off, kv.second});
        std::sort(own_sorted.begin(), own_sorted.end());
        own_sufmin.assign(own_sorted.size(), 0);
        int m = (int)ops.size();
        for (size_t p = own_sorted.size(); p-- > 0;) { m = std::min(m, own_sorted[p].second); own_sufmin[p] = m; }
        size_t pos = own_sorted.size();
        for (int i = (int)ops.size() - 1; i >= 0; --i) {
            while (pos > 0 && own_sufmin[pos - 1] >= i) --pos;
            const int64_t lo = pos < own_sorted.size() ? own_sorted[pos].first : n_train;
            for (auto& kv : owner)
                if (kv.first->off >= lo && kv.second < i)
                    throw P3dError("gradient bucket order broken at op " + ops[i].name + " / variable " + kv.first->name);
        }
        if (pos != 0) throw P3dError("gradient bucket walk does not reach offset 0");
        adam_split = 0;
        size_t q = own_sorted.size();
        while (q > 0 && own_sufmin[q - 1] >= 1) --q;
        int64_t read_end = 0;
        for (auto& a : acts)
            if (a.stem_link)
                for (const Param* p : a.stem_link->reads) read_end = std::max(read_end, p->off + p->count);
        while (q < own_sorted.size() && own_sorted[q].first < read_end) ++q;
        if (q > 0 && q < own_sorted.size() && (own_sorted[q].first & 3) == 0) adam_split = own_sorted[q].first;
    }

    void tune_plans() {
        Ctx c; c.training = true; c.s = stream;
        const bool want = fuse_bn;
        const bool want_bwd = fuse_bn_bwd;
        for (int mode = 0; mode < 3; ++mode) {
            fuse_bn = mode >= 1; fuse_bn_bwd = mode == 2;
            run_forward(c);
            run_loss(c);
            run_backward(c, false);
        }
        fuse_bn = want; fuse_bn_bwd = want_bwd;
        HIPCHECK(hipStreamSynchronize(c.s));
        HIPCHECK(fill_async(flat_g, 0, (size_t)n_train * sizeof(float), c.s, "gradients"));
        HIPCHECK(hipStreamSynchronize(c.s));
        pred_ready = false;
    }

    void plan_zero_arenas() {
        for (int phase = 0; phase < 2; ++phase) {
            std::vector<std::pair<float*, size_t>> reqs;
            Ctx c; c.training = true; c.s = stream; c.dry = &reqs;
            if (phase == 0) { for (auto& op : ops) op.fwd(c); }
            else { for (int i = (int)ops.size() - 1; i >= 0; --i) ops[i].bwd(c); }
            std::vector<std::pair<Act*, bool>> movers;
            size_t total = 0;
            for (auto& rq : reqs)
                for (auto& a : acts) {
                    if (a.parent || !a.views.empty()) continue;
                    const size_t bytes = (size_t)a.rows() * a.C * sizeof(float);
                    if (bytes != rq.second) continue;
                    const bool is_g = (a.g == rq.first), is_p = (a.p == rq.first);
                    if (!is_g && !is_p) continue;
                    movers.push_back({&a, is_g});
                    total += (bytes + 255) / 256 * 256;
                    break;
                }
            if (!total) continue;
            char* base = (char*)dalloc<char>((int64_t)total);
            size_t off = 0;
            for (auto& mv : movers) {
                float*& ptr = mv.second ? mv.first->g : mv.first->p;
                ptr = (float*)(base + off);
                off += ((size_t)mv.first->rows() * mv.first->C * sizeof(float) + 255) / 256 * 256;
            }
            if (phase == 0) { zf = base; zf_bytes = total; } else { zb = base; zb_bytes = total; }
        }
    }
```

### sap3d_tensorflow_amd/csrc/net_sched.inc

```
    void debug_sync(const char* dir, const Op& op, const Ctx& c) {
        if (!runtime_env().debug_sync) return;
        fprintf(stderr, "[p3d] %s %s (%s) ...", dir, op.name.c_str(), op.kind.c_str());
        fflush(stderr);
        HIPCHECK(hipStreamSynchronize(c.s));
        fprintf(stderr, " ok\n");
        fflush(stderr);
    }
    void run_forward(const Ctx& c) {
        sib_pending.clear();
        if (stats_count) HIPCHECK(fill_async(stats_arena, 0, (size_t)stats_count * sizeof(double), c.s, "statistics"));
        if (zf_bytes) HIPCHECK(fill_async(zf, 0, zf_bytes, c.s, "forward-arena"));
        Ctx cz = c; cz.z0 = zf; cz.z1 = zf + zf_bytes;
        cz.fuse = fuse_bn && !c.per_sample && !c.dry;
        last_forward_fused = cz.fuse;
        if (!c.dry) pred_ready = true;
        const bool no_side_f = runtime_env().no_side_stream;
        cz.side = (c.prof || no_side_f || c.dry) ? nullptr : side_stream;
        const Ctx& c2 = cz;
        for (auto& op : ops) {
            if (c.prof) c.prof->cur_op = op.name;
            op.fwd(c2);
            debug_sync("fwd", op, c);
        }
    }
    LossArgs loss_args() const {
        return {loss_kind, logits->p, pred->p, d_y, (long)pred->rows(), head_sigmoid ? 1 : 0, d_loss, d_dlogits};
    }
    void run_loss(const Ctx& c) {
        HIPCHECK(fill_async(d_loss, 0, sizeof(double), c.s, "loss"));
        if (!c.dry) last_loss_kind = loss_kind;
        if (loss_kind == P3D_LOSS_KLD_CC) return run_map_loss(c);
        if (loss_kind == P3D_LOSS_SALIENCY) return run_saliency_loss(c);
        const LossArgs a = loss_args();
        const LaunchDesc d = p3d_loss_desc(a);
        launch(c, d.kernel, d.flops, d.bytes, [&]() { return p3d_loss(a, c.s); });
    }
    void run_map_loss(const Ctx& c) {
        const double rows = (double)pred->rows();
        const int ts = head_sigmoid ? 1 : 0;
        const double sg = ts ? 0.0 : 3.0;
        const MapLossArgs a = p3d_map_loss_args(logits->p, pred->p, d_y, (long long)pred->N * pred->D, (long long)pred->H * pred->W, ts,
                                                kld_weight, cc_weight, d_loss, d_dlogits, d_map_scratch, d_map_cnt);
        launch(c, "map_loss_sums_kernel", rows * (2.0 + sg), rows * 8.0, [&]() { return p3d_map_loss_launch(0, a, c.s); });
        launch(c, "map_loss_terms_kernel", rows * (18.0 + sg), rows * 8.0, [&]() { return p3d_map_loss_launch(1, a, c.s); });
        launch(c, "map_loss_grad_kernel", rows * (20.0 + sg), rows * 12.0, [&]() { return p3d_map_loss_launch(2, a, c.s); });
    }
    bool saliency_needs_fixations() const { return loss_kind == P3D_LOSS_SALIENCY && sal_nss > 0.f; }
    void check_fixations(bool fresh) const {
        if (!saliency_needs_fixations()) return;
        if (!d_fix) throw P3dError("the loss has an NSS term (w_nss > 0) and no fixation maps were uploaded: p3d_upload_fixations");
        if (fresh && !fix_fresh)
            throw P3dError("the loss has an NSS term (w_nss > 0) and the fixation maps are those of an earlier batch: "
                           "p3d_upload_fixations before every p3d_train_step / p3d_backward");
    }
    SaliencyLossArgs saliency_loss_args() const {
        return p3d_saliency_loss_args(logits->p, pred->p, d_y, d_fix, (long long)pred->N * pred->D, (long long)pred->H * pred->W,
                                      head_sigmoid ? 1 : 0, sal_kld, sal_cc, sal_nss, sal_sim, d_loss, d_dlogits, d_sal_scratch, d_sal_cnt);
    }
    void run_saliency_loss(const Ctx& c) {
        check_fixations(false);
        if (!d_sal_scratch) throw P3dError("saliency loss: scratch was not planned (p3d_set_loss)");
        const double rows = (double)pred->rows();
        const double sg = head_sigmoid ? 0.0 : 3.0, fb = sal_nss > 0.f ? 1.0 : 0.0;
        const SaliencyLossArgs a = saliency_loss_args();
        launch(c, "saliency_loss_sums_kernel", rows * (8.0 + sg), rows * (8.0 + fb), [&]() { return p3d_saliency_loss_launch(0, a, c.s); });
        launch(c, "saliency_loss_terms_kernel", rows * (24.0 + sg), rows * 8.0, [&]() { return p3d_saliency_loss_launch(1, a, c.s); });
        launch(c, "saliency_loss_grad_kernel", rows * (32.0 + sg), rows * (12.0 + fb), [&]() { return p3d_saliency_loss_launch(2, a, c.s); });
    }
    bool zeroed_early = false;
    hipEvent_t ev_zeroed = nullptr, ev_zero_fork = nullptr;
    void zero_backward_arenas(hipStream_t st, bool with_zb) {
        if (with_zb && zb_bytes) HIPCHECK(fill_async(zb, 0, zb_bytes, st, "backward-arena"));
        HIPCHECK(fill_async(flat_g, 0, (size_t)n_train * sizeof(float), st, "gradients"));
        if (red_count) HIPCHECK(fill_async(red_arena, 0, (size_t)red_count * sizeof(double), st, "reductions"));
    }
    void zero_early(const Ctx& c) {
        if (runtime_env().no_side_stream || !side_stream || c.prof || c.dry) return;
        if (!ev_zeroed) HIPCHECK(hipEventCreateWithFlags(&ev_zeroed, local_event_flags()));
        if (!ev_zero_fork) HIPCHECK(hipEventCreateWithFlags(&ev_zero_fork, local_event_flags()));
        HIPCHECK(ev_record(ev_zero_fork, c.s));
        HIPCHECK(ev_wait(side_stream, ev_zero_fork));
        zero_backward_arenas(side_stream, false);
        HIPCHECK(ev_record(ev_zeroed, side_stream));
        zeroed_early = true;
    }
    bool run_backward(const Ctx& c0, bool allreduce, bool with_adam = false) {
        Ctx c = c0; c.z0 = zb; c.z1 = zb + zb_bytes;
        c.fuse = last_forward_fused && !c.dry;
        c.fuse_bwd = c.fuse && fuse_bn_bwd;
        bool adam_done = false;
        const bool no_side = runtime_env().no_side_stream;
        c.side = (c.prof || no_side) ? nullptr : side_stream;
        if (zeroed_early) {
            zeroed_early = false;
            HIPCHECK(ev_wait(c.s, ev_zeroed));
            if (zb_bytes) HIPCHECK(fill_async(zb, 0, zb_bytes, c.s, "backward-arena"));
        } else {
            zero_backward_arenas(c.s, true);
        }
        for (auto& a : acts) if (a.stem_link) a.stem_link->pending = false;
        int64_t hi = n_train;
        size_t own_pos = own_sorted.size();
        wq.clear(); wq_flushes = 0;
        std::vector<std::pair<hipEvent_t, std::function<void(const Ctx&)>>> parked;
        bool early_adam = false, early_comm = false;
        const bool finish_main = c.acc_finish && !(allreduce && comm && !bucket_hook);
        static const bool no_defer = p3d_tune_env("P3D_DEFER_SIDE") && atoi(p3d_tune_env("P3D_DEFER_SIDE")) == 0;
        const bool defer_on = c.side && !no_defer && defer_release_op > 0 && defer_budget > 0;
        parked_flops = 0;
        auto release_parked = [&]() {
            c.defer = nullptr;
            bool first = true;
            for (auto& job : parked) {
                if (first || !c.side) on_side_stream(c, job.first, job.second);
                else { Ctx sc = c; sc.s = c.side; job.second(sc); }
                first = false;
            }
            parked.clear();
        };
        for (int i = (int)ops.size() - 1; i >= 0; --i) {
            if (c.prof) c.prof->cur_op = ops[i].name;
            c.bwd_op = ops[i].name.c_str();
            if (i == 1) flush_wgrads(c);
            if (i == 0 && adam_split > 0 && adam_split < n_train && c.side && !c.dry) {
                flush_wgrads(c);
                if (c.defer || !parked.empty()) release_parked();
                const bool reduce = allreduce && (comm || bucket_hook);
                if (hi > adam_split) {
                    if (reduce) reduce_range(adam_split, hi, c, 1);
                    hi = adam_split;
                }
                static const bool no_split = p3d_tune_env("P3D_SPLIT_ADAM") && atoi(p3d_tune_env("P3D_SPLIT_ADAM")) == 0;
                if (with_adam && !no_split) {
                    HIPCHECK(ev_record(ev_side_early, c.side));
                    early_comm = reduce && comm && !bucket_hook;
                    if (early_comm) HIPCHECK(ev_record(ev_comm_early, comm_stream));
                    early_adam = true;
                }
            }
            if (defer_on) {
                if (i > defer_release_op) c.defer = parked_flops < defer_budget ? &parked : nullptr;
                else if (c.defer || !parked.empty()) release_parked();
            }
            ops[i].bwd(c);
            debug_sync("bwd", ops[i], c);
            if (early_adam) {
                early_adam = false;
                HIPCHECK(ev_wait(c.s, ev_side_early));
                if (early_comm) HIPCHECK(ev_wait(c.s, ev_comm_early));
                if (finish_main) grad_accum_range(c, GACC_FINISH, adam_split, n_train);
                if (clip_on()) {
                    sumsq_range(c, adam_split, n_train);
                } else {
                    adam_begin(c);
                    adam_range(c, adam_split, n_train);
                }
                adam_done = true;
            }
            {
                while (own_pos > 0 && own_sufmin[own_pos - 1] >= i) --own_pos;
                const int64_t lo = own_pos < own_sorted.size() ? own_sorted[own_pos].first : n_train;
                if ((hi > lo && hi - lo >= bucket_floats) || i == 0) {
                    const int64_t start = (i == 0) ? 0 : lo;
                    flush_wgrads(c);
                    if (i == 0 && (c.defer || !parked.empty())) release_parked();
                    if (parked.empty()) {
                        if (hi > start && allreduce && (comm || bucket_hook)) reduce_range(start, hi, c, i);
                        hi = start;
                    }
                }
            }
        }
        flush_wgrads(c);
        if (c.defer || !parked.empty()) release_parked();
        for (auto& a : acts)
            if (a.stem_link && a.stem_link->pending) {
                a.stem_link->pending = false;
                throw P3dError("the stem BatchNorm's backward left its apply pass to a filter gradient that never ran (" + a.name + ")");
            }
        static const bool tune_tail = p3d_tune_env("P3D_TUNE_TAIL") != nullptr;
        static hipEvent_t tail_main = nullptr, tail_side = nullptr;
        if (tune_tail && c.side && !c.dry) {
            if (!tail_main) { HIPCHECK(hipEventCreate(&tail_main)); HIPCHECK(hipEventCreate(&tail_side)); }
// ... 536 lines not shown
```

### sap3d_tensorflow_amd/csrc/p3d_kernels.h

```cpp
#pragma once
#include <vector>
#include <hip/hip_runtime.h>
#include <stdint.h>

#define P3D_MAX_TAPS 27
#ifndef P3D_WGRAD_GROUP
#define P3D_WGRAD_GROUP 6
#endif
#define P3D_STAT_REPLICAS 16
#define P3D_FOLD_MAX 32

#include <stdlib.h>
inline const char* p3d_tune_env(const char* name) {
#if defined(P3D_TUNING)
    return getenv(name);
#else
    (void)name;
    return nullptr;
#endif
}

struct P3dFastDiv { unsigned mul; int shift; };
inline P3dFastDiv p3d_fastdiv(unsigned d) {
    P3dFastDiv f{0u, 0};
// ... 43 lines not shown
    int16_t dd, dh, dw;
    int16_t widx;
};

struct BnFold {
    const float* gamma; const float* beta;
    const float* part; int nparts;
    int C;
    float* scale; float* shift; float* mean; float* invstd;
    float* moving_mean; float* moving_var;
    double inv_m;
    float eps; int publish; int update_moving;
};
struct BnGradFold {
    const float* gamma; const float* mean; const float* invstd;
    const float* part; int nparts;
    int C;
    float* coef;
    float* dgamma; float* dbeta;
    double inv_m; int publish;
};
struct BnGate {
    const float* y; int ldy;
    const float* scale; const float* shift; const float* mean; const float* invstd;
    float* out; int ldo;
    float* part;
};
enum { P3D_AT_NONE = 0, P3D_AT_RELU1 = 1, P3D_AT_RELU2 = 2, P3D_AT_GRAD = 3 };

struct IgemmArgs {
    const float* x;
    int N, Di, Hi, Wi;
    int ldx;
    int K;
    int Gd, Gh, Gw;
    P3dFastDiv fGd, fGh, fGw;
    int isd, ish, isw;
    float* y;
    int Do, Ho, Wo;
    int ldy;
    int Nc;
    int osd, osh, osw, ood, ooh, oow;
    const float* w;
    int wT;
    const float* bias;
    float* statpart;
    int stat_base;
    int accum;
    const float* zeros;
    float* slab; unsigned* cnt; int nsplit;
    int f16;
    int xcd_min_tiles;
    int at_mode;
    const float* x2; int ldx2;
    BnFold f1, f2;
    BnGradFold gf;
    int ngate, raw_store;
    BnGate gate[2];
    int ntaps;
    P3dTap taps[P3D_MAX_TAPS];
};

#define P3D_IGEMM_CLASSES 8
struct IgemmClass {
    int Gd, Gh, Gw;
    P3dFastDiv fGd, fGh, fGw;
    int ood, ooh, oow;
    int stat_base;
    int ntaps;
    int blk0;
    const float* w; const float* bias; float* y; float* statpart;
    int nsplit;
    int tile0;
    int ntiles;
    long long slab0, cnt0;
    P3dTap taps[P3D_MAX_TAPS];
};
struct IgemmGroupArgs {
    IgemmArgs common;
    int nclass;
    IgemmClass cls[P3D_IGEMM_CLASSES];
};

struct P3dIgemmPlan {
    int bm = 64, bn = 64, splits = 1;
    const char* name = "";
    int stream_blocks = 0;
};
inline int p3d_igemm2_mtiles(const IgemmArgs& a, const P3dIgemmPlan& pl) {
    if (pl.stream_blocks > 0) return pl.stream_blocks;
    const long long M = (long long)a.N * a.Gd * a.Gh * a.Gw;
    return (int)((M + pl.bm - 1) / pl.bm);
}
hipError_t p3d_stream_scratch(hipStream_t s, size_t slab_floats, size_t counters, float** slab, unsigned** cnt);
long long p3d_scratch_dirty_counters();
void p3d_release_scratch();

struct WgradArgs {
    const float* x;
    int N, Di, Hi, Wi, ldx, K;
    int Gd, Gh, Gw;
    int isd, ish, isw;
    const float* dy;
    int ldy, Nc;
    float* dw;
    float* dbias;
    int ksplit;
    int greedy;
    int polite;
    int pair;
    const float* zeros;
    int xt;
    const float* x2; int ldx2;
    const float* xs1; const float* xt1; const float* xs2; const float* xt2;
    int dyt;
    const float* dy2; int ldy2;
    const float* dcoef;
    int ntaps;
    P3dTap taps[P3D_MAX_TAPS];
};

#ifdef __cplusplus
extern "C++" {
#endif

P3dIgemmPlan p3d_igemm2_plan(const IgemmArgs& a, int allow_split);
void p3d_tune_begin(hipStream_t s);
void p3d_tune_end();
hipError_t p3d_launch_igemm2(const IgemmArgs& a, const P3dIgemmPlan& plan, hipStream_t s);
bool p3d_igemm2_tail_split(const IgemmArgs& a, const P3dIgemmPlan& pl);
bool p3d_igemm2_groupable(const IgemmArgs* v, int n, const P3dIgemmPlan& plan);
hipError_t p3d_launch_igemm2_group(const IgemmArgs* v, int n, const P3dIgemmPlan& plan, hipStream_t s);
void p3d_igemm2_override(int tile, int splits);
int p3d_pw_stream_blocks(const IgemmArgs& a);
int p3d_pw_stream_max_blocks(long long M, int N);
hipError_t p3d_launch_pw_stream(const IgemmArgs& a, hipStream_t s);
hipError_t p3d_launch_wgrad2(const WgradArgs& a, hipStream_t s);
hipError_t p3d_launch_wgrad2_group(const WgradArgs* probs, int n, hipStream_t s);
const char* p3d_wgrad2_variant(const WgradArgs& a);
const char* p3d_wgrad2_group_variant(const WgradArgs* probs, int n, bool fused);
int p3d_wgrad2_group_cuts(const WgradArgs* probs, int n, int* cuts, int* kstride, int* tm, int* tn);
void p3d_wgrad2_force_tile(int tm, int tn);

struct BnParams {
    const float* gamma; const float* beta;
    float* moving_mean; float* moving_var;
    const float* statpart;
    int nparts;
    float* scale; float* shift;
    float* mean; float* invstd;
    int C;
};
hipError_t p3d_bn_finalize(const BnParams& bn, long M, int use_batch, int update_moving, float eps, hipStream_t s);
int p3d_bn_stats_parts(long M, int C);
hipError_t p3d_bn_stats(const float* y, int ld, long M, int C, float* statpart, hipStream_t s);

hipError_t p3d_bn_grad_finalize(const BnGradFold& f, hipStream_t s);

struct BnApplyArgs {
    int mode;
    long M; int C;
    const float* y1; int ld1; const float* scale1; const float* shift1;
    const float* y2; int ld2; const float* scale2; const float* shift2;
    float* z; int ldz;
    float drop_scale;
    float drop_rate; unsigned long long seed;
    const unsigned long long* seed_dev;
};
hipError_t p3d_bn_apply(const BnApplyArgs& a, hipStream_t s);
bool p3d_bn_fold_apply_ok(long M, int C, int nparts1, int nparts2, float drop_scale);
hipError_t p3d_bn_fold_apply(const BnApplyArgs& a, const BnParams& bn1, const BnParams& bn2, int batch1, int batch2, int update_moving,
                             float eps, hipStream_t s);

struct BnBwdArgs {
    int mode;
    long M; int C;
    const float* dz; int lddz;
    const float* y1; int ld1; const float* scale1; const float* shift1; const float* mean1; const float* invstd1;
    const float* y2; int ld2; const float* scale2; const float* shift2; const float* mean2; const float* invstd2;
    const float* gamma1; const float* gamma2;
    float* part1; float* part2;
    int nparts;
    float* coef1; float* coef2;
    float* dgamma1; float* dbeta1; float* dgamma2; float* dbeta2;
    int batch1, batch2;
    float* dy1; int lddy1; int acc1;
    float* dy2; int lddy2; int acc2;
    float drop_scale; float drop_rate; unsigned long long seed; const unsigned long long* seed_dev;
};
int p3d_bn_bwd_parts(long M, int C);
hipError_t p3d_bn_bwd_reduce(const BnBwdArgs& a, hipStream_t s);
hipError_t p3d_bn_bwd_finalize(const BnBwdArgs& a, hipStream_t s);
hipError_t p3d_bn_bwd_apply(const BnBwdArgs& a, hipStream_t s);

struct BnSmallArgs {
    int mode; int M; int C;
    const float* y1; int ld1;
    const float* y2; int ld2;
    BnParams bn1, bn2;
    int batch1, batch2;
    int update_moving; float eps;
    float* z; int ldz;
    const float* dz; int lddz;
    float* dy1; int lddy1;
    float* dy2; int lddy2; int acc2;
    float* dgamma1; float* dbeta1; float* dgamma2; float* dbeta2;
};
bool p3d_bn_small_ok(long M, int C);
hipError_t p3d_bn_small_fwd(const BnSmallArgs& a, hipStream_t s);
hipError_t p3d_bn_small_bwd(const BnSmallArgs& a, hipStream_t s);

struct GnParams {
    const float* gamma; const float* beta;
    double* sums;
    float* scale; float* shift; float* mean; float* invstd;
// ... 609 lines not shown
```

### sap3d_tensorflow_amd/ops.py

```python
import ctypes as C

import numpy as np

from ._lib import LOSSES, OPTIMIZERS, check, fptr, lib


def _f32(a):
    return np.ascontiguousarray(a, dtype=np.float32)


def _shape5(s):
    return (C.c_int64 * 5)(*[int(v) for v in s])


def _i3(s):
    return (C.c_int * 3)(*[int(v) for v in s])


def _same_out(size, s):
    return -(-size // s)


def _strides3(strides):
    strides = list(strides)
# ... 608 lines not shown
    photo = np.ascontiguousarray([[r[6], r[7]] for r in d], dtype=np.float32)
    xo, yo = np.empty_like(x), np.empty_like(y)
    check(lib().p3d_debug_augment(device, fptr(x), fptr(y), f.ctypes.data_as(u8) if f is not None else None, B, T, H, W,
                                  geom.ctypes.data_as(C.POINTER(C.c_int32)), fptr(photo), int(offset), fptr(xo), fptr(yo),
                                  fo.ctypes.data_as(u8) if fo is not None else None))
    return xo, yo, fo


def augment_draw(seed, g, H, W, flip=0., reverse=0., min_scale=1., contrast=0., brightness=0.):
    from ._lib import P3dAugment
    cfg = P3dAugment(float(flip), float(reverse), float(min_scale), float(contrast), float(brightness))
    geom, photo = (C.c_int32 * 6)(), (C.c_float * 2)()
    check(lib().p3d_debug_augment_draw(int(seed), int(g), int(H), int(W), C.byref(cfg), geom, photo))
    return (bool(geom[0]), bool(geom[1]), geom[2], geom[3], geom[4], geom[5], np.float32(photo[0]), np.float32(photo[1]))


def optimizer_decay(kind, p, g, m, tiles, lr=1e-4, momentum=0.9, use_nesterov=False, lr_on_device=False, update=True, offset=0,
                    device=0, gscale=None):
    k = _opt_kind(kind)
    p, g, m = (_f32(a).ravel().copy() for a in (p, g, m))
    if not (p.size == g.size == m.size):
        raise ValueError("p, g, m differ in size")
    if gscale is not None:
        if not update:
            raise ValueError("gscale: the gradient-only launch scales nothing")
        term, _ = _opt_scaled(k, p, g, m, np.zeros_like(p), tiles, 1, lr, 0.0, 0.0, 0.0, momentum, use_nesterov, lr_on_device, gscale,
                              offset, device)
        return g, p, m, term
    lens = np.array([int(n) for n, _ in tiles], np.int64)
    offs = np.concatenate([[0], np.cumsum(lens)[:-1]]).astype(np.int64)
    cs = np.array([c for _, c in tiles], np.float32)
    i64 = C.POINTER(C.c_int64)
    term = C.c_double()
    check(lib().p3d_debug_optimizer_decay(device, k, fptr(p), fptr(g), fptr(m), p.size, int(offset), offs.ctypes.data_as(i64),
                                          lens.ctypes.data_as(i64), fptr(cs), len(tiles), float(lr), float(momentum),
                                          1 if use_nesterov else 0, 1 if lr_on_device else 0, 1 if update else 0, C.byref(term)))
    return g, p, m, term.value


GRAD_NORM_CHUNK = 8192


def grad_norm(g, clip_norm, p=None, tiles=None, ranges=None, offset=0, blocks=0, device=0):
    g = _f32(g).ravel()
    n = g.size
    if p is not None:
        p = _f32(p).ravel()
        if p.size != n:
            raise ValueError("g and p differ in size")
    if tiles is None:
        tiles = [(min(GRAD_NORM_CHUNK, n - a), 0.0) for a in range(0, n, GRAD_NORM_CHUNK)]
    offs, lens, cs, at = [], [], [], 0
    for length, c in tiles:
        if c is not None:
            offs.append(at); lens.append(int(length)); cs.append(c)
        at += int(length)
    if at != n:
        raise ValueError("tiles must cover [0, n)")
    offs, lens, cs = np.array(offs, np.int64), np.array(lens, np.int64), np.array(cs, np.float32)
    ranges = [(0, n)] if ranges is None else list(ranges)
    lo = np.array([int(a) for a, _ in ranges], np.int64)
    hi = np.array([int(b) for _, b in ranges], np.int64)
    i64 = C.POINTER(C.c_int64)
    ss, nm, sc = C.c_double(), C.c_double(), C.c_float()
    check(lib().p3d_debug_grad_norm(device, fptr(g), fptr(p), n, int(offset), offs.ctypes.data_as(i64), lens.ctypes.data_as(i64),
                                    fptr(cs), len(offs), lo.ctypes.data_as(i64), hi.ctypes.data_as(i64), len(ranges),
                                    float(np.float32(clip_norm)), int(blocks), C.byref(ss), C.byref(nm), C.byref(sc)))
    return ss.value, nm.value, np.float32(sc.value)


def stat_parts(xshape, fshape, strides, transpose=False):
    w, c = C.c_int(), C.c_int()
    check(lib().p3d_debug_stat_parts(_shape5(xshape), _shape5(fshape), _i3(_strides3(strides)), 1 if transpose else 0,
                                     C.byref(w), C.byref(c)))
    return w.value, c.value


def igemm_groupable(xshape, fshape, strides):
    r = lib().p3d_debug_igemm_groupable(_shape5(xshape), _shape5(fshape), _i3(_strides3(strides)))
    check(-1 if r < 0 else 0)
    return bool(r)


def bias_add_grad(dy, device=0):
    g = _f32(dy)
    c = g.shape[-1]
    out = np.empty((c,), np.float32)
    check(lib().p3d_op_bias_add_grad(device, fptr(g), g.size // c if c else 0, c, fptr(out)))
    return out


def attention_core(g, f, h, d_o=None, device=0):
    g, f, h = _f32(g), _f32(f), _f32(h)
    B, ng, ci = g.shape
    nf, ch = h.shape[1], h.shape[2]
    if f.shape != (B, nf, ci) or h.shape[0] != B or ci * 8 != ch:
        raise ValueError("attention_core: g [B,Ng,ch/8], f [B,Nf,ch/8], h [B,Nf,ch]")
    o = np.empty((B, ng, ch), np.float32)
    if d_o is None:
        check(lib().p3d_op_attention_core(device, B, ng, nf, ch, fptr(g), fptr(f), fptr(h), fptr(o), None, None, None, None))
        return o
    d = _f32(d_o)
    if d.shape != o.shape:
        raise ValueError("attention_core: d_o has the shape of o")
    dg, df, dh = np.empty_like(g), np.empty_like(f), np.empty_like(h)
    check(lib().p3d_op_attention_core(device, B, ng, nf, ch, fptr(g), fptr(f), fptr(h), fptr(o), fptr(d), fptr(dg), fptr(df), fptr(dh)))
    return o, dg, df, dh


ATTENTION_MODES = {"stored": 1, "flash": 2}


def attention_core_launch(mode, g, f, h, d_o=None, device=0):
    g, f, h = _f32(g), _f32(f), _f32(h)
    B, ng, ci = g.shape
    nf, ch = h.shape[1], h.shape[2]
    if f.shape != (B, nf, ci) or h.shape[0] != B or ci * 8 != ch:
        raise ValueError("attention_core_launch: g [B,Ng,ch/8], f [B,Nf,ch/8], h [B,Nf,ch]")
    m = ATTENTION_MODES[mode]
    o = np.empty((B, ng, ch), np.float32)
    if d_o is None:
        check(lib().p3d_debug_attention_core(device, m, B, ng, nf, ch, fptr(g), fptr(f), fptr(h), fptr(o), None, None, None, None))
        return o
    d = _f32(d_o)
    if d.shape != o.shape:
        raise ValueError("attention_core_launch: d_o has the shape of o")
    dg, df, dh = np.empty_like(g), np.empty_like(f), np.empty_like(h)
    check(lib().p3d_debug_attention_core(device, m, B, ng, nf, ch, fptr(g), fptr(f), fptr(h), fptr(o), fptr(d), fptr(dg), fptr(df),
                                         fptr(dh)))
    return o, dg, df, dh


def attention_splits(B, ng, nf, ch):
    sp = (C.c_int * 4)()
    check(lib().p3d_debug_attention_splits(B, ng, nf, ch, sp))
    return tuple(sp)


def softmax_rows_launch(s, cols, d=None, guard_rows=0, device=0):
    s = _f32(s).copy()
    rows, ld = s.shape[0] - guard_rows, s.shape[1]
    if d is None:
        check(lib().p3d_debug_softmax_rows(device, 0, rows, cols, ld, fptr(s), None, guard_rows))
        return s
    d = _f32(d).copy()
    if d.shape != s.shape:
        raise ValueError("softmax_rows_launch: d has the shape of s")
    check(lib().p3d_debug_softmax_rows(device, 1, rows, cols, ld, fptr(s), fptr(d), guard_rows))
    return d


def attn_mix(r, x, gamma, C_, offset=(0, 0, 0), drop_rate=0.0, seed=0, seed_dev=False, z=None, dz=None, accx=False, dr=None, dx=None,
             dgamma=0.0, device=0):
    r, x = _f32(r), _f32(x)
    M = r.shape[0]
    z = np.full((M, int(C_)), np.nan, np.float32) if z is None else _f32(z).copy()
    args = (device, M, int(C_), fptr(r), r.shape[1], int(offset[0]), fptr(x), x.shape[1], int(offset[1]), float(gamma), float(drop_rate),
            int(seed), 1 if seed_dev else 0, fptr(z), z.shape[1], int(offset[2]))
    if dz is None:
        check(lib().p3d_debug_attn_mix(*args, None, 0, None, None, None))
        return z
    dz = _f32(dz)
    dr = np.full(r.shape, np.nan, np.float32) if dr is None else _f32(dr).copy()
    dx = np.full(x.shape, np.nan, np.float32) if dx is None else _f32(dx).copy()
    dgm = np.array([dgamma], np.float32)
    if dz.shape != z.shape or dr.shape != r.shape or dx.shape != x.shape:
# ... 20 lines not shown
```

Measured before the change: 537.0.

## Merge sibling convs' input-gradient igemms into one split-K pair kernel

Adds a pair igemm kernel that computes the input gradients of two sibling convolutions, which share an input, in a single launch. Each operand's taps and K steps become separate split-K slices, and the two partial sums are folded through the shared slab reduction. In backward, the first sibling's dgrad is parked and launched together with the second's. The aim is to remove one launch and the extra read-modify-write of dx, and to fill the GPU better on small grids. The cost is more bookkeeping state and a planner that only merges 64x64 tiles under row and tile limits.

```diff
diff --git a/include/p3d_hip.h b/include/p3d_hip.h
--- a/include/p3d_hip.h
+++ b/include/p3d_hip.h
@@ -210,6 +210,11 @@
                         int nrange, float clip_norm, int max_blocks, double* sumsq, double* norm, float* scale);
 int p3d_debug_stat_parts(const int64_t xshape[5], const int64_t wshape[5], const int s[3], int transpose, int* written, int* cap);
 int p3d_debug_igemm_groupable(const int64_t xshape[5], const int64_t wshape[5], const int s[3]);
+int p3d_debug_pair_plan(const int64_t xshape0[5], const int64_t xshape1[5], int cout, const int k0[3], const int k1[3], int total,
+                        int* nslices, int* ranges, const char** why);
+int p3d_debug_pair_dgrad(int device, const float* dy0, const float* w0, const int k0[3], const float* dy1, const float* w1, const int k1[3],
+                         const int64_t xshape[5], int cout, int accum, int total, float* dx, char* kernels, int kernels_cap, int* nslices,
+                         int reps, float* usec);
 int p3d_op_max_pool3d(int device, const float* x, const int64_t xshape[5], const int ksize[3], const int s[3], float* y);
 int p3d_op_max_pool3d_grad(int device, const float* x, const int64_t xshape[5], const int ksize[3], const int s[3],
                            const float* dy, float* dx);
diff --git a/sap3d_tensorflow_amd/csrc/conv_igemm2.hip b/sap3d_tensorflow_amd/csrc/conv_igemm2.hip
--- a/sap3d_tensorflow_amd/csrc/conv_igemm2.hip
+++ b/sap3d_tensorflow_amd/csrc/conv_igemm2.hip
@@ -50,6 +50,7 @@
     int achunk[LA];
     int t, kc;
     int issued;
+    const float* x;
 };
 template <int LB>
 struct BLoad {
@@ -81,6 +82,7 @@
         }
     }
     st.t = s_begin / kchunks; st.kc = s_begin - st.t * kchunks; st.issued = 0;
+    st.x = geo.x;
 }
 template <int BN, bool WT>
 __device__ __forceinline__ void b_init(const IgemmArgs& p, const float* w, BLoad<BN / 32>& st, int n0, int wave, int lane, int s_begin, int kchunks) {
@@ -116,7 +118,7 @@
         const bool ok = st.base[i] >= 0 && (unsigned)id < (unsigned)p.Di && (unsigned)ih < (unsigned)p.Hi &&
                         (unsigned)iw < (unsigned)p.Wi;
         const long long row = (long long)st.base[i] + ((long long)id * p.Hi + ih) * p.Wi + iw;
-        st.aptr[i] = ok ? p.x + row * p.ldx + st.achunk[i] : nullptr;
+        st.aptr[i] = ok ? st.x + row * p.ldx + st.achunk[i] : nullptr;
         if (TWO) st.aptr2[TWO ? i : 0] = ok ? p.x2 + row * p.ldx2 + st.achunk[i] : nullptr;
     }
 }
@@ -453,8 +455,9 @@
     }
 }
 
-template <int BM, int BN, bool WT, bool F16, int AT>
-__device__ __forceinline__ void igemm2_body(const IgemmArgs& p, const Geo& geo, const int tile_id, const int slice) {
+template <int BM, int BN, bool WT, bool F16, int AT, bool PAIR = false>
+__device__ __forceinline__ void igemm2_body(const IgemmArgs& p, const Geo& geo, const int tile_id, const int slice, const int s_begin,
+                                            const int s_end) {
     constexpr int TM = BM / 64, TN = BN / 64;
     constexpr int LA = BM / 32;
     using L = Lds<BM, BN, AT>;
@@ -499,10 +502,6 @@
             rowIdx[r] = ro;
         }
     };
-    const int total_steps = geo.ntaps * kchunks;
-    const int per = (total_steps + nsplit - 1) / nsplit;
-    const int s_begin = slice * per;
-    const int s_end = min(total_steps, s_begin + per);
     const int nsteps = max(s_end - s_begin, 0);
 
     f32x16 acc[TM][TN];
@@ -604,26 +603,38 @@
                 const int i = tid + (i0 + q) * 256;
                 const int r = i / F4R, c4 = (i - r * F4R) * 4;
                 src[q] = slabs + r * BN + c4;
-                v[q] = *reinterpret_cast<const float4*>(src[q]);
             }
-            int sidx = 1;
-            for (; sidx + 3 < nsplit; sidx += 4) {
-                float4 a[4][4];
-#pragma unroll
-                for (int t = 0; t < 4; ++t)
-#pragma unroll
-                    for (int q = 0; q < 4; ++q) a[t][q] = *reinterpret_cast<const float4*>(src[q] + (size_t)(sidx + t) * (BM * BN));
-#pragma unroll
-                for (int t = 0; t < 4; ++t)
-#pragma unroll
-                    for (int q = 0; q < 4; ++q) { v[q].x += a[t][q].x; v[q].y += a[t][q].y; v[q].z += a[t][q].z; v[q].w += a[t][q].w; }
-            }
-            for (; sidx < nsplit; ++sidx) {
-                float4 a[4];
-#pragma unroll
-                for (int q = 0; q < 4; ++q) a[q] = *reinterpret_cast<const float4*>(src[q] + (size_t)sidx * (BM * BN));
-#pragma unroll
-                for (int q = 0; q < 4; ++q) { v[q].x += a[q].x; v[q].y += a[q].y; v[q].z += a[q].z; v[q].w += a[q].w; }
+            auto fold_run = [&](const int first, const int last, float4 (&w)[4]) {
+#pragma unroll
+                for (int q = 0; q < 4; ++q) w[q] = *reinterpret_cast<const float4*>(src[q] + (size_t)first * (BM * BN));
+                int sidx = first + 1;
+                for (; sidx + 3 < last; sidx += 4) {
+                    float4 a[4][4];
+#pragma unroll
+                    for (int t = 0; t < 4; ++t)
+#pragma unroll
+                        for (int q = 0; q < 4; ++q) a[t][q] = *reinterpret_cast<const float4*>(src[q] + (size_t)(sidx + t) * (BM * BN));
+#pragma unroll
+                    for (int t = 0; t < 4; ++t)
+#pragma unroll
+                        for (int q = 0; q < 4; ++q) { w[q].x += a[t][q].x; w[q].y += a[t][q].y; w[q].z += a[t][q].z; w[q].w += a[t][q].w; }
+                }
+                for (; sidx < last; ++sidx) {
+                    float4 a[4];
+#pragma unroll
+                    for (int q = 0; q < 4; ++q) a[q] = *reinterpret_cast<const float4*>(src[q] + (size_t)sidx * (BM * BN));
+#pragma unroll
+                    for (int q = 0; q < 4; ++q) { w[q].x += a[q].x; w[q].y += a[q].y; w[q].z += a[q].z; w[q].w += a[q].w; }
+                }
+            };
+            if constexpr (!PAIR) {
+                fold_run(0, nsplit, v);
+            } else {
+                float4 u[4];
+                fold_run(0, geo.nsplit0, u);
+                fold_run(geo.nsplit0, nsplit, v);
+#pragma unroll
+                for (int q = 0; q < 4; ++q) { v[q].x += u[q].x; v[q].y += u[q].y; v[q].z += u[q].z; v[q].w += u[q].w; }
             }
 #pragma unroll
             for (int q = 0; q < 4; ++q) {
@@ -642,6 +653,13 @@
     if (T < min_tiles) return b;
     const int x = b & 7, q = T >> 3, r = T & 7;
     return x * q + min(x, r) + (b >> 3);
+}
+
+__device__ __forceinline__ void even_cut(int K, int ntaps, int nsplit, int slice, int& s_begin, int& s_end) {
+    const int total_steps = ntaps * ((K + BK - 1) / BK);
+    const int per = (total_steps + nsplit - 1) / nsplit;
+    s_begin = slice * per;
+    s_end = min(total_steps, s_begin + per);
 }
 
 template <int BM, int BN, bool WT, bool F16 = false, int AT = 0>
@@ -650,10 +668,12 @@
     Geo geo;
     geo.Gd = p.Gd; geo.Gh = p.Gh; geo.Gw = p.Gw; geo.fGd = p.fGd; geo.fGh = p.fGh; geo.fGw = p.fGw;
     geo.ood = p.ood; geo.ooh = p.ooh; geo.oow = p.oow; geo.stat_base = p.stat_base; geo.ntaps = p.ntaps; geo.taps = p3d_kernarg_taps(offsetof(IgemmArgs, taps));
-    geo.w = p.w; geo.bias = p.bias; geo.y = p.y; geo.statpart = p.statpart;
+    geo.x = p.x; geo.w = p.w; geo.bias = p.bias; geo.y = p.y; geo.statpart = p.statpart;
     geo.nsplit = p.nsplit; geo.slab = p.slab; geo.cnt = p.cnt;
     const int tile = p.nsplit == 1 ? xcd_tile((int)blockIdx.x, (int)gridDim.x, p.xcd_min_tiles) : (int)blockIdx.x;
-    igemm2_body<BM, BN, WT, F16, AT>(p, geo, tile, (int)blockIdx.y);
+    int s_begin, s_end;
+    even_cut(p.K, p.ntaps, p.nsplit, (int)blockIdx.y, s_begin, s_end);
+    igemm2_body<BM, BN, WT, F16, AT>(p, geo, tile, (int)blockIdx.y, s_begin, s_end);
 }
 template <int BM, int BN, bool WT, bool F16 = false>
 __global__ __launch_bounds__(256) void igemm2_group_kernel(const IgemmGroupArgs g) {
@@ -666,14 +686,36 @@
     geo.Gd = g.cls[c].Gd; geo.Gh = g.cls[c].Gh; geo.Gw = g.cls[c].Gw; geo.fGd = g.cls[c].fGd; geo.fGh = g.cls[c].fGh; geo.fGw = g.cls[c].fGw;
     geo.ood = g.cls[c].ood; geo.ooh = g.cls[c].ooh; geo.oow = g.cls[c].oow; geo.stat_base = g.cls[c].stat_base; geo.ntaps = g.cls[c].ntaps;
     geo.taps = p3d_kernarg_taps(offsetof(IgemmGroupArgs, cls) + (size_t)c * sizeof(IgemmClass) + offsetof(IgemmClass, taps));
-    geo.w = g.cls[c].w; geo.bias = g.cls[c].bias; geo.y = g.cls[c].y; geo.statpart = g.cls[c].statpart;
+    geo.x = g.common.x; geo.w = g.cls[c].w; geo.bias = g.cls[c].bias; geo.y = g.cls[c].y; geo.statpart = g.cls[c].statpart;
     const int tile0 = g.cls[c].tile0;
     geo.nsplit = g.cls[c].nsplit;
     geo.slab = g.common.slab + (g.cls[c].slab0 - (long long)tile0 * geo.nsplit * (BM * BN));
     geo.cnt = g.common.cnt + (g.cls[c].cnt0 - tile0);
     const int local = (int)blockIdx.x - g.cls[c].blk0;
     const int tile = geo.nsplit == 1 ? xcd_tile(local, g.cls[c].ntiles, g.common.xcd_min_tiles) : local / geo.nsplit;
-    igemm2_body<BM, BN, WT, F16, 0>(g.common, geo, tile0 + tile, local % geo.nsplit);
+    int s_begin, s_end;
+    even_cut(g.common.K, geo.ntaps, geo.nsplit, local % geo.nsplit, s_begin, s_end);
+    igemm2_body<BM, BN, WT, F16, 0>(g.common, geo, tile0 + tile, local % geo.nsplit, s_begin, s_end);
+}
+
+template <int BM, int BN, bool WT>
+__global__ __launch_bounds__(256) void igemm2_pair_kernel(const IgemmPairArgs g) {
+    p3d_warm_kernargs<IgemmPairArgs>();
+    const IgemmArgs& p = g.common;
+    const int gs = (int)blockIdx.y;
+    const bool second = gs >= g.nslices0;
+    Geo geo;
+    geo.Gd = p.Gd; geo.Gh = p.Gh; geo.Gw = p.Gw; geo.fGd = p.fGd; geo.fGh = p.fGh; geo.fGw = p.fGw;
+    geo.ood = p.ood; geo.ooh = p.ooh; geo.oow = p.oow; geo.stat_base = 0;
+    geo.ntaps = second ? g.ntaps1 : p.ntaps;
+    geo.taps = p3d_kernarg_taps(second ? offsetof(IgemmPairArgs, taps1) : offsetof(IgemmPairArgs, common) + offsetof(IgemmArgs, taps));
+    geo.x = second ? g.x1 : p.x; geo.w = second ? g.w1 : p.w;
+    geo.bias = nullptr; geo.y = p.y; geo.statpart = nullptr;
+    geo.nsplit = g.nslices0 + g.nslices1; geo.nsplit0 = g.nslices0; geo.slab = p.slab; geo.cnt = p.cnt;
+    const int steps = geo.ntaps * ((p.K + BK - 1) / BK);
+    int s_begin, s_end;
+    p3d_pair_slice_range(steps, second ? g.nslices1 : g.nslices0, second ? gs - g.nslices0 : gs, &s_begin, &s_end);
+    igemm2_body<BM, BN, WT, false, 0, true>(p, geo, (int)blockIdx.x, gs, s_begin, s_end);
 }
 
 constexpr int MAX_TABLE_FLOATS = 4 * 2048;
@@ -1013,3 +1055,84 @@
     if (pl.bm == 128 && pl.bn == 64) return launch_group_t<128, 64>(g, tiles, s);
     return launch_group_t<64, 64>(g, tiles, s);
 }
+
+static void pair_split(int steps0, int steps1, int total, int* n) {
+    total = std::max(2, std::min(total, steps0 + steps1));
+    int n1 = (int)((2ll * total * steps1 + (steps0 + steps1)) / (2ll * (steps0 + steps1)));
+    n1 = std::max(1, std::min(n1, total - 1));
+    n1 = std::max(total - steps0, std::min(n1, steps1));
+    n[0] = total - n1; n[1] = n1;
+}
+
+P3dPairPlan p3d_igemm2_pair_plan(const IgemmArgs* v, int total) {
+    P3dPairPlan pp;
+    auto refuse = [&](const char* why) { pp.merged = false; pp.why = why; return pp; };
+    const IgemmArgs &a = v[0], &b = v[1];
+    for (int i = 0; i < 2; ++i)
+        if (v[i].at_mode != P3D_AT_NONE || v[i].ngate || v[i].statpart || v[i].bias || v[i].f16 || v[i].ntaps < 1)
+            return refuse("operand transform, gate, statistics, bias, fp16 or no taps");
+    if (a.N != b.N || a.Gd != b.Gd || a.Gh != b.Gh || a.Gw != b.Gw || a.Do != b.Do || a.Ho != b.Ho || a.Wo != b.Wo ||
+        a.osd != b.osd || a.osh != b.osh || a.osw != b.osw || a.ood != b.ood || a.ooh != b.ooh || a.oow != b.oow || a.y != b.y ||
+        a.ldy != b.ldy || a.Nc != b.Nc)
+        return refuse("different output grids, strides or outputs");
+    if (a.Di != b.Di || a.Hi != b.Hi || a.Wi != b.Wi || a.isd != b.isd || a.ish != b.ish || a.isw != b.isw || a.ldx != b.ldx ||
+        a.K != b.K || a.wT != b.wT)
+        return refuse("different gathered extents, strides or channel counts");
+    const P3dIgemmPlan q0 = p3d_igemm2_plan(a, 1), q1 = p3d_igemm2_plan(b, 1);
+    if (q0.stream_blocks > 0 || q1.stream_blocks > 0) return refuse("streaming plan");
+    if (q0.bm != q1.bm || q0.bn != q1.bn) return refuse("different tile shapes");
+    if (q0.bm != 64 || q0.bn != 64) return refuse("tile shape other than 64x64");
+    const long long M = (long long)a.N * a.Gd * a.Gh * a.Gw;
+    const long long tiles = ((M + 63) / 64) * ((a.Nc + 63) / 64);
+    if (total == 0 && M < P3D_PAIR_MIN_ROWS) return refuse("fewer rows than P3D_PAIR_MIN_ROWS");
+    if (total == 0 && tiles > P3D_PAIR_MAX_TILES) return refuse("more tiles than P3D_PAIR_MAX_TILES");
+    const int kchunks = (a.K + BK - 1) / BK;
+    const int steps0 = a.ntaps * kchunks, steps1 = b.ntaps * kchunks;
+    if (total >= 2) {
+        pair_split(steps0, steps1, total, pp.nslices);
+    } else {
+        pp.nslices[0] = std::max(1, std::min(q0.splits, steps0));
+        pp.nslices[1] = std::max(1, std::min(q1.splits, steps1));
+    }
+    pp.bm = 64; pp.bn = 64;
+    pp.merged = true;
+    return pp;
+}
+
+hipError_t p3d_launch_igemm2_pair(const IgemmArgs* v, const P3dPairPlan& pp, hipStream_t s) {
+    if (!pp.merged || pp.bm != 64 || pp.bn != 64 || pp.nslices[0] < 1 || pp.nslices[1] < 1) return hipErrorInvalidValue;
+    if (!p3d_igemm2_pair_plan(v, pp.nslices[0] + pp.nslices[1]).merged) return hipErrorInvalidValue;
+    IgemmPairArgs g;
+    memset(&g, 0, sizeof(g));
+    g.common = v[0];
+    IgemmArgs& a = g.common;
+    const int kchunks = (a.K + BK - 1) / BK;
+    if (pp.nslices[0] > a.ntaps * kchunks || pp.nslices[1] > v[1].ntaps * kchunks) return hipErrorInvalidValue;
+    const long long M = (long long)a.N * a.Gd * a.Gh * a.Gw;
+    if (M <= 0 || a.Nc <= 0) return hipSuccess;
+    if (M >= (1ll << 31) || (long long)a.N * a.Di * a.Hi * a.Wi >= (1ll << 31) || (long long)a.N * a.Do * a.Ho * a.Wo >= (1ll << 31))
+        return hipErrorInvalidValue;
+    if (a.Gd * a.isd >= 1024 || a.Gh * a.ish >= 1024 || a.Gw * a.isw >= 1024 || a.ntaps > P3D_MAX_TAPS || v[1].ntaps > P3D_MAX_TAPS)
+        return hipErrorInvalidValue;
+    if ((a.K & 3) || (a.ldx & 3) || !a.zeros || (a.Nc & 3) || (a.ldy & 3) || !a.x || !v[1].x || !a.w || !v[1].w) return hipErrorInvalidValue;
+    a.fGd = p3d_fastdiv((unsigned)a.Gd); a.fGh = p3d_fastdiv((unsigned)a.Gh); a.fGw = p3d_fastdiv((unsigned)a.Gw);
+    g.x1 = v[1].x; g.w1 = v[1].w; g.ntaps1 = v[1].ntaps;
+    for (int t = 0; t < v[1].ntaps; ++t) g.taps1[t] = v[1].taps[t];
+    g.nslices0 = pp.nslices[0]; g.nslices1 = pp.nslices[1];
+    const int S = g.nslices0 + g.nslices1;
+    const long long tiles = ((M + 63) / 64) * ((a.Nc + 63) / 64);
+    if (tiles >= 65536ll * 32768 || S > 65535) return hipErrorInvalidValue;
+    a.nsplit = S; a.xcd_min_tiles = xcd_min_tiles();
+    const hipError_t e = p3d_stream_scratch(s, (size_t)tiles * S * 64 * 64, (size_t)tiles, &a.slab, &a.cnt);
+    if (e != hipSuccess) return e;
+    constexpr size_t sm = smem_fixed_bytes<64, 64, 0>();
+    static std::once_flag once;
+    std::call_once(once, [] {
+        hipFuncSetAttribute((const void*)igemm2_pair_kernel<64, 64, false>, hipFuncAttributeMaxDynamicSharedMemorySize, (int)sm);
+        hipFuncSetAttribute((const void*)igemm2_pair_kernel<64, 64, true>, hipFuncAttributeMaxDynamicSharedMemorySize, (int)sm);
+    });
+    const dim3 grid((unsigned)tiles, (unsigned)S), blk(256);
+    if (a.wT) hipLaunchKernelGGL((igemm2_pair_kernel<64, 64, true>), grid, blk, sm, s, g);
+    else hipLaunchKernelGGL((igemm2_pair_kernel<64, 64, false>), grid, blk, sm, s, g);
+    return hipGetLastError();
+}
diff --git a/sap3d_tensorflow_amd/csrc/igemm_epilogue.h b/sap3d_tensorflow_amd/csrc/igemm_epilogue.h
--- a/sap3d_tensorflow_amd/csrc/igemm_epilogue.h
+++ b/sap3d_tensorflow_amd/csrc/igemm_epilogue.h
@@ -16,8 +16,10 @@
     P3dFastDiv fGd, fGh, fGw;
     int ood, ooh, oow, stat_base, ntaps;
     P3dKTap* taps;
+    const float* x;
     const float* w; const float* bias; float* y; float* statpart;
     int nsplit; float* slab; unsigned* cnt;
+    int nsplit0;
 };
 
 __device__ __forceinline__ float4 shfl_xor4(float4 v, int o) {
diff --git a/sap3d_tensorflow_amd/csrc/net.hip b/sap3d_tensorflow_amd/csrc/net.hip
--- a/sap3d_tensorflow_amd/csrc/net.hip
+++ b/sap3d_tensorflow_amd/csrc/net.hip
@@ -372,6 +372,17 @@
     }
     for (auto& q : v) launch_igemm(c, q, 1);
     return false;
+}
+const char* const kPairKernelName = "igemm2_pair_kernel<64,64>";
+void pair_prepare(IgemmArgs& a, int accum) { a.zeros = g_zero_page; a.accum = accum; a.statpart = nullptr; a.stat_base = 0; }
+void launch_igemm_pair(const Ctx& c, const IgemmArgs* pair, const P3dPairPlan& pp) {
+    double f0, b0, f1, b1;
+    igemm_work(pair[0], f0, b0);
+    IgemmArgs second = pair[1];
+    second.accum = 0;
+    igemm_work(second, f1, b1);
+    b1 -= 4.0 * (double)second.N * second.Gd * second.Gh * second.Gw * second.Nc;
+    launch(c, kPairKernelName, f0 + f1, b0 + b1, [&]() { return p3d_launch_igemm2_pair(pair, pp, c.s); });
 }
 
 float adam_step_size(float lr, float b1, float b2, int64_t t_step) {
@@ -1376,6 +1387,9 @@
     }
 
     std::vector<IgemmArgs> sib_pending;
+    struct SibGrad { ConvGeo g; Act* y = nullptr; Param* w = nullptr; int Cout = 0; };
+    std::shared_ptr<SibGrad> sib_build;
+    std::vector<IgemmArgs> sib_bwd_pending;
 
 #include "net_ops.inc"
 #include "net_gn.inc"
diff --git a/sap3d_tensorflow_amd/csrc/net_abi.inc b/sap3d_tensorflow_amd/csrc/net_abi.inc
--- a/sap3d_tensorflow_amd/csrc/net_abi.inc
+++ b/sap3d_tensorflow_amd/csrc/net_abi.inc
@@ -812,6 +812,7 @@
     c.z0 = h->zb; c.z1 = h->zb + h->zb_bytes;
     HIPCHECK(hipMemcpy2DAsync(b->g, (size_t)b->ld * 4, dout, (size_t)b->C * 4, (size_t)b->C * 4, (size_t)b->rows(), hipMemcpyHostToDevice, c.s));
     h->wq.clear(); h->wq_flushes = 0; h->parked_flops = 0;
+    h->sib_bwd_pending.clear();
     for (size_t i = it->second.op1; i-- > it->second.op0;) {
         c.bwd_op = h->ops[i].name.c_str();
         h->ops[i].bwd(c);
@@ -2023,6 +2024,94 @@
         if (v.empty()) splits[0] = splits[1] = 0;
     }
     dout.get(out, rout * ld_out);
+    API_END
+}
+
+namespace {
+IgemmArgs pair_member(const int64_t xs[5], int cout, const int k[3], const float* dy, const float* w, float* dx, int accum) {
+    if (cout < 4 || (cout & 3) || xs[4] < 4 || (xs[4] & 3)) throw P3dError("pair: channel counts are multiples of 4");
+    const int64_t ws[5] = {k[0], k[1], k[2], xs[4], cout};
+    const int one[3] = {1, 1, 1};
+    const ConvProblem p = conv_problem(xs, ws, one, 0);
+    auto v = p.input_gradient(dy, w, dx, 0, 0, accum);
+    if (v.size() != 1) throw P3dError("pair: a stride-1 conv has one input-gradient launch");
+    pair_prepare(v[0], accum);
+    return v[0];
+}
+}
+
+int p3d_debug_pair_plan(const int64_t xs0[5], const int64_t xs1[5], int cout, const int k0[3], const int k1[3], int total, int* nslices,
+                        int* ranges, const char** why) {
+    try {
+        if (!xs0 || !k0 || !k1 || !nslices || !ranges) throw P3dError("null argument");
+        if (total < 0 || total > 16) throw P3dError("pair_plan: total is 0 (the step's rule), 1 (its slices at any size) or 2..16");
+        static float dummy[4];
+        const IgemmArgs pair[2] = {pair_member(xs0, cout, k0, dummy, dummy, dummy + 2, 0),
+                                   pair_member(xs1 ? xs1 : xs0, cout, k1, dummy + 1, dummy + 1, dummy + 2, 1)};
+        const P3dPairPlan pp = p3d_igemm2_pair_plan(pair, total);
+        if (why) *why = pp.why;
+        nslices[0] = nslices[1] = 0;
+        if (!pp.merged) return 0;
+        if (pp.nslices[0] > 16 || pp.nslices[1] > 16) throw P3dError("pair_plan: more than 16 slices in a class");
+        const int kchunks = (cout + 31) / 32;
+        for (int c = 0; c < 2; ++c) {
+            nslices[c] = pp.nslices[c];
+            for (int i = 0; i < pp.nslices[c]; ++i)
+                p3d_pair_slice_range(pair[c].ntaps * kchunks, pp.nslices[c], i, ranges + (c * 16 + i) * 2, ranges + (c * 16 + i) * 2 + 1);
+        }
+        return 1;
+    } catch (const std::exception& e) {
+        g_err = e.what();
+        return -1;
+    }
+}
+
+int p3d_debug_pair_dgrad(int device, const float* dy0, const float* w0, const int k0[3], const float* dy1, const float* w1, const int k1[3],
+                         const int64_t xs[5], int cout, int accum, int total, float* dx, char* kernels, int kernels_cap, int* nslices,
+                         int reps, float* usec) {
+    API_BEGIN
+    HIPCHECK(hipSetDevice(device));
+    if (!dy0 || !w0 || !k0 || !dy1 || !w1 || !k1 || !xs || !dx) throw P3dError("null argument");
+    if (total < -1 || total > 16) throw P3dError("pair_dgrad: total is -1 (two launches), 0 (the step's rule), 1 (merged, its slices) or 2..16");
+    if (reps < 0 || reps > 1000 || (reps && !usec)) throw P3dError("pair_dgrad: reps in [0, 1000], with a place for the time");
+    const int64_t rows = xs[0] * xs[1] * xs[2] * xs[3], nx = rows * xs[4], ny = rows * cout;
+    const int64_t nw0 = (int64_t)k0[0] * k0[1] * k0[2] * xs[4] * cout, nw1 = (int64_t)k1[0] * k1[1] * k1[2] * xs[4] * cout;
+    DevBuf d0(ny, dy0), d1(ny, dy1), f0(nw0, w0), f1(nw1, w1), out(nx, dx);
+    ensure_zero_page();
+    IgemmArgs pair[2] = {pair_member(xs, cout, k0, d0.p, f0.p, out.p, accum ? 1 : 0), pair_member(xs, cout, k1, d1.p, f1.p, out.p, 1)};
+    P3dPairPlan pp;
+    if (total >= 0) {
+        pp = p3d_igemm2_pair_plan(pair, total);
+        if (!pp.merged && total > 0) throw P3dError(std::string("pair_dgrad: the pair cannot be merged: ") + pp.why);
+    }
+    if (nslices) { nslices[0] = pp.merged ? pp.nslices[0] : 0; nslices[1] = pp.merged ? pp.nslices[1] : 0; }
+    Ctx c;
+    const auto send = [&]() {
+        if (pp.merged) { launch_igemm_pair(c, pair, pp); return; }
+        std::vector<IgemmArgs> a{pair[0]}, b{pair[1]};
+        run_igemm_group(c, a, accum != 0, nullptr);
+        run_igemm_group(c, b, true, nullptr);
+    };
+    std::string names;
+    traced_kernels(send, names);
+    put_string(names, kernels, kernels_cap);
+    out.get(dx, nx);
+    if (reps) {
+        hipEvent_t e0 = nullptr, e1 = nullptr;
+        HIPCHECK(hipEventCreate(&e0));
+        HIPCHECK(hipEventCreate(&e1));
+        try {
+            for (int i = 0; i < 5; ++i) send();
+            HIPCHECK(hipEventRecord(e0, c.s));
+            for (int i = 0; i < reps; ++i) send();
+            HIPCHECK(hipEventRecord(e1, c.s));
+            HIPCHECK(hipEventSynchronize(e1));
+            float ms = 0.f;
+            HIPCHECK(hipEventElapsedTime(&ms, e0, e1));
+            *usec = ms * 1000.f / (float)reps;
+        } catch (...) { hipEventDestroy(e0); hipEventDestroy(e1); throw; }
+        hipEventDestroy(e0); hipEventDestroy(e1);
+    }
     API_END
 }
 
diff --git a/sap3d_tensorflow_amd/csrc/net_ops.inc b/sap3d_tensorflow_amd/csrc/net_ops.inc
--- a/sap3d_tensorflow_amd/csrc/net_ops.inc
+++ b/sap3d_tensorflow_amd/csrc/net_ops.inc
@@ -91,6 +91,36 @@
             }
             return wa;
         };
+        std::shared_ptr<SibGrad> partner;
+        if (sibling == 1) {
+            sib_build = std::make_shared<SibGrad>();
+            sib_build->g = g; sib_build->y = y; sib_build->w = w; sib_build->Cout = Cout;
+        } else if (sibling == 2) {
+            partner.swap(sib_build);
+        }
+        const auto pair_input_gradient = [=](const Ctx& c, IgemmArgs a, int accum) {
+            if (sibling == 2) {
+                if (!sib_bwd_pending.empty()) throw P3dError("sibling conv " + opname + ": an earlier pair never sent its input gradients");
+                if (!partner || !partner->y->g) return false;
+                auto vp = igemm_conv_input_side(partner->g, x->N, partner->y->g, partner->y->ld, partner->Cout, x->g, x->ld, Cin,
+                                                partner->w->p, nullptr, 1, false);
+                if (vp.size() != 1) return false;
+                IgemmArgs pair[2] = {a, vp[0]};
+                pair_prepare(pair[0], accum); pair_prepare(pair[1], 1);
+                if (!p3d_igemm2_pair_plan(pair, 0).merged) return false;
+                sib_bwd_pending.push_back(pair[0]);
+                return true;
+            }
+            if (sib_bwd_pending.empty()) return false;
+            if (sib_bwd_pending.size() != 1 || accum != 1) throw P3dError("sibling conv " + opname + ": its pair's parked input gradient does not fit");
+            IgemmArgs pair[2] = {sib_bwd_pending[0], a};
+            sib_bwd_pending.clear();
+            pair_prepare(pair[1], 1);
+            const P3dPairPlan pp = p3d_igemm2_pair_plan(pair, 0);
+            if (!pp.merged) throw P3dError("sibling conv " + opname + ": the planner no longer merges the pair it parked (" + pp.why + ")");
+            launch_igemm_pair(c, pair, pp);
+            return true;
+        };
         op.bwd = [=](const Ctx& c) {
             if (!(c.fuse_bwd && cf.any())) {
                 queue_wgrad(c, wgrad_args(c.fuse && cf.at != 0));
@@ -99,6 +129,7 @@
                     auto v = igemm_conv_input_side(g, x->N, y->g, y->ld, Cout, x->g, x->ld, Cin, w->p, nullptr, accum,
                                                    !accum);
                     if (f16()) for (auto& a : v) a.f16 = 1;
+                    if (sibling && v.size() == 1 && pair_input_gradient(c, v[0], accum)) return;
                     run_igemm_group(c, v, accum != 0, nullptr);
                 }
                 return;
diff --git a/sap3d_tensorflow_amd/csrc/net_plan.inc b/sap3d_tensorflow_amd/csrc/net_plan.inc
--- a/sap3d_tensorflow_amd/csrc/net_plan.inc
+++ b/sap3d_tensorflow_amd/csrc/net_plan.inc
@@ -91,7 +91,7 @@
             std::vector<std::pair<float*, size_t>> reqs;
             Ctx c; c.training = true; c.s = stream; c.dry = &reqs;
             if (phase == 0) { for (auto& op : ops) op.fwd(c); }
-            else { for (int i = (int)ops.size() - 1; i >= 0; --i) ops[i].bwd(c); }
+            else { sib_bwd_pending.clear(); for (int i = (int)ops.size() - 1; i >= 0; --i) ops[i].bwd(c); }
             std::vector<std::pair<Act*, bool>> movers;
             size_t total = 0;
             for (auto& rq : reqs)
diff --git a/sap3d_tensorflow_amd/csrc/net_sched.inc b/sap3d_tensorflow_amd/csrc/net_sched.inc
--- a/sap3d_tensorflow_amd/csrc/net_sched.inc
+++ b/sap3d_tensorflow_amd/csrc/net_sched.inc
@@ -99,6 +99,7 @@
             zero_backward_arenas(c.s, true);
         }
         for (auto& a : acts) if (a.stem_link) a.stem_link->pending = false;
+        sib_bwd_pending.clear();
         int64_t hi = n_train;
         size_t own_pos = own_sorted.size();
         wq.clear(); wq_flushes = 0;
diff --git a/sap3d_tensorflow_amd/csrc/p3d_kernels.h b/sap3d_tensorflow_amd/csrc/p3d_kernels.h
--- a/sap3d_tensorflow_amd/csrc/p3d_kernels.h
+++ b/sap3d_tensorflow_amd/csrc/p3d_kernels.h
@@ -149,6 +149,30 @@
     IgemmClass cls[P3D_IGEMM_CLASSES];
 };
 
+struct IgemmPairArgs {
+    IgemmArgs common;
+    const float* x1; const float* w1;
+    int ntaps1;
+    int nslices0, nslices1;
+    P3dTap taps1[P3D_MAX_TAPS];
+};
+#if defined(__HIPCC__)
+__host__ __device__
+#endif
+inline void p3d_pair_slice_range(int steps, int nslices, int slice, int* begin, int* end) {
+    const int q = steps / nslices, r = steps - q * nslices;
+    *begin = slice * q + (slice < r ? slice : r);
+    *end = *begin + q + (slice < r ? 1 : 0);
+}
+#define P3D_PAIR_MIN_ROWS 256
+#define P3D_PAIR_MAX_TILES 255
+struct P3dPairPlan {
+    bool merged = false;
+    int bm = 64, bn = 64;
+    int nslices[2] = {0, 0};
+    const char* why = "";
+};
+
 struct P3dIgemmPlan {
     int bm = 64, bn = 64, splits = 1;
     const char* name = "";
@@ -198,6 +222,8 @@
 bool p3d_igemm2_tail_split(const IgemmArgs& a, const P3dIgemmPlan& pl);
 bool p3d_igemm2_groupable(const IgemmArgs* v, int n, const P3dIgemmPlan& plan);
 hipError_t p3d_launch_igemm2_group(const IgemmArgs* v, int n, const P3dIgemmPlan& plan, hipStream_t s);
+P3dPairPlan p3d_igemm2_pair_plan(const IgemmArgs* v, int total);
+hipError_t p3d_launch_igemm2_pair(const IgemmArgs* v, const P3dPairPlan& plan, hipStream_t s);
 void p3d_igemm2_override(int tile, int splits);
 int p3d_pw_stream_blocks(const IgemmArgs& a);
 int p3d_pw_stream_max_blocks(long long M, int N);
diff --git a/sap3d_tensorflow_amd/ops.py b/sap3d_tensorflow_amd/ops.py
--- a/sap3d_tensorflow_amd/ops.py
+++ b/sap3d_tensorflow_amd/ops.py
@@ -714,6 +714,33 @@
     return bool(r)
 
 
+def pair_plan(xshape, cout, k0, k1, total=0, xshape1=None):
+    ns = (C.c_int * 2)()
+    ranges = (C.c_int * 64)()
+    why = C.c_char_p()
+    r = lib().p3d_debug_pair_plan(_shape5(xshape), _shape5(xshape1) if xshape1 is not None else None, int(cout), _i3(k0), _i3(k1),
+                                  int(total), ns, ranges, C.byref(why))
+    check(-1 if r < 0 else 0)
+    cuts = [[(ranges[(c * 16 + i) * 2], ranges[(c * 16 + i) * 2 + 1]) for i in range(ns[c])] for c in range(2)]
+    return bool(r), cuts, (why.value or b"").decode()
+
+
+def pair_dgrad(dy0, w0, dy1, w1, dx=None, total=0, reps=0, device=0):
+    dy0, w0, dy1, w1 = _f32(dy0), _f32(w0), _f32(dy1), _f32(w1)
+    xshape = tuple(dy0.shape[:4]) + (w0.shape[3],)
+    cout = w0.shape[4]
+    if dy1.shape != dy0.shape or w1.shape[3:] != w0.shape[3:] or dy0.shape[4] != cout:
+        raise ValueError("pair_dgrad: both convs map [N,D,H,W,C] to [N,D,H,W,cout]")
+    out = np.zeros(xshape, np.float32) if dx is None else _f32(dx).reshape(xshape).copy()
+    names = C.create_string_buffer(512)
+    ns = (C.c_int * 2)()
+    usec = C.c_float()
+    check(lib().p3d_debug_pair_dgrad(device, fptr(dy0), fptr(w0), _i3(w0.shape[:3]), fptr(dy1), fptr(w1), _i3(w1.shape[:3]),
+                                     _shape5(xshape), int(cout), 0 if dx is None else 1, int(total), fptr(out), names, 512, ns,
+                                     int(reps), C.byref(usec)))
+    return out, names.value.decode().split(";"), (ns[0], ns[1]), (usec.value if reps else None)
+
+
 def bias_add_grad(dy, device=0):
     g = _f32(dy)
     c = g.shape[-1]
```

Result: no change. 541.3 (median of 6 runs) (+0.8%).
